# kurtkuehnert/bevy_terrain

Hardware: AMD Instinct MI355X
Metric: terrain tiles/sec preprocessed (16k^2 heightmap) (higher is better)
Workload: dtype f32; 1 GPU; synthetic 16384x16384 fBm R16 heightmap (seed 42), T=512, b=2, lod_count=6: split + pyramid + stitch into 1365 tiles; jobs_in_flight=1, ranks_seen=1, all_gather_bytes_per_rank=0

## Files before the change

bevy_terrain_amd/csrc/bt_fused.hip:

```cpp
#include <cstdio>
#include <cstdlib>
#include <type_traits>

#include "bt_internal.hpp"

namespace bt {

namespace {

constexpr uint32_t kInvalid = 0xFFFFFFFFu;

#include "bt_stitch.hpp"

#ifdef BT_DEBUG_HOOKS
#define BT_ABLATE(A, bits) ((A).ablate & (bits))
#else
#define BT_ABLATE(A, bits) 0u
#endif
constexpr uint32_t kMainRows = 8;
#ifndef BT_DMA_POS
#define BT_DMA_POS 0
#endif

constexpr uint32_t kDmaPos = BT_DMA_POS;
constexpr uint32_t kMaxBorder = 8;

struct MainItem {
    uint32_t side, x, y, atlas_index, raster;
};

struct FusedArgs {
    AttachmentMeta m;
    uint16_t* atlas;
    const RasterDev* rasters;
    const MainItem* items;
    const uint32_t* grids;
    uint32_t grid_lod_lo, grid_lod_hi, grid_sides;
    uint32_t regular, reg_first;
    const TaskDev* seam_tasks;
    uint32_t seam_count, seam_skip;
    uint32_t seam_pull;
    uint32_t tail_extras;
    float tlx, tly, brx, bry;
    uint32_t lod;
    uint32_t levels;
    uint32_t item_count;
    uint32_t groups;
    uint32_t sides;
    uint32_t lds_pitch;
    uint32_t lds_rows;
    uint32_t apron_lods;
    uint32_t rotate_priority;
    uint32_t apron_cols;
    uint32_t prev_zero;
    uint32_t apron_global;
    uint32_t single_buffer;
    uint32_t ablate;
};

__device__ __forceinline__ float unorm16_to_float(uint32_t t) {
    const float x = float(t);
    const float r = 1.0f / 65535.0f;
    const float q0 = x * r;
    const float e = __builtin_fmaf(-q0, 65535.0f, x);
    return __builtin_fmaf(e, r, q0);
}
__device__ __forceinline__ uint32_t float_to_unorm16(float e) {
    const float cl = __builtin_amdgcn_fmed3f(e, 0.0f, 1.0f);
    return uint32_t(0.5f + 65535.0f * cl);
}
__device__ __forceinline__ float mixf(float a, float b, float t) { return a * (1.0f - t) + b * t; }

struct Axis {
    int i0, i1;
    float fr;
};

__host__ __device__ __forceinline__ Axis split_axis(uint32_t r, uint32_t c, uint32_t tile, float scale, float lo, float hi, uint32_t dim) {
    const float tc = float(r) / float(c);
    const float s = (float(tile) + tc) / scale;
    const float u = (s - lo) / (hi - lo);
    const float q = u * float(dim) - 0.5f;
    const float fl = floorf(q);
    Axis a;
    a.fr = q - fl;
    const int i = int(fl);
    const int last = int(dim) - 1;
    const int j = i + 1;
    a.i0 = i < 0 ? 0 : (i > last ? last : i);
    a.i1 = j < 0 ? 0 : (j > last ? last : j);
    return a;
}

__device__ __forceinline__ uint32_t grid_lookup(const FusedArgs& A, uint32_t side, uint32_t lod, int x, int y) {
    const int n = int(1u << lod);
    if (x < 0 || y < 0 || x >= n || y >= n) return kInvalid;
    if (lod < A.grid_lod_lo || lod > A.grid_lod_hi || side >= A.grid_sides) return kInvalid;
    if (A.regular) {
        const uint32_t hi4 = 4u << (2u * A.grid_lod_hi);
        return A.reg_first + side * ((hi4 - (1u << (2u * A.grid_lod_lo))) / 3u) + (hi4 - (4u << (2u * lod))) / 3u + uint32_t(x) * uint32_t(n) + uint32_t(y);
    }
    const uint32_t lo4 = 1u << (2u * A.grid_lod_lo), per_side = ((4u << (2u * A.grid_lod_hi)) - lo4) / 3u;
    const uint32_t off = side * per_side + ((1u << (2u * lod)) - lo4) / 3u;
    return A.grids[off + uint32_t(x) * uint32_t(n) + uint32_t(y)];
}

struct TileNb {
    uint32_t self, n, e, s, w;
};

__device__ __forceinline__ TileNb load_tile_nb(const FusedArgs& A, uint32_t side, uint32_t lod, uint32_t x, uint32_t y) {
    const int ix = int(x), iy = int(y);
    TileNb t;
    t.self = grid_lookup(A, side, lod, ix, iy);
    t.n = grid_lookup(A, side, lod, ix, iy - 1);
    t.e = grid_lookup(A, side, lod, ix + 1, iy);
    t.s = grid_lookup(A, side, lod, ix, iy + 1);
    t.w = grid_lookup(A, side, lod, ix - 1, iy);
    return t;
}

template <bool kCentre = true, typename TT = uint16_t>
__device__ __forceinline__ void push_pixel(const FusedArgs& A, uint32_t side, uint32_t lod, uint32_t tx, uint32_t ty,
                                           uint32_t self_index, uint32_t cx, uint32_t cy, TT v) {
    const uint32_t T = A.m.texture_size, b = A.m.border_size, c = A.m.center_size;
    const uint64_t tile_texels = uint64_t(T) * T;
    TT* atlas = reinterpret_cast<TT*>(A.atlas);
    TT* self = atlas + uint64_t(self_index) * tile_texels;
    if (kCentre) self[uint64_t(b + cy) * T + b + cx] = v;
    const int ex = cx < b ? -1 : (cx >= c - b ? 1 : 0);
    const int ey = cy < b ? -1 : (cy >= c - b ? 1 : 0);
    if (ex == 0 && ey == 0) return;
    const uint32_t o = b + c;
    const int ix = int(tx), iy = int(ty);
    const uint32_t ax = uint32_t(int(b + cx) - ex * int(c)), ay = uint32_t(int(b + cy) - ey * int(c));
    const int nn = int(1u << lod);
    auto cross_face = [&](int x, int y) { return A.seam_pull != 0 && ((x < 0 || x >= nn) != (y < 0 || y >= nn)); };
    if (ex != 0) {
        const uint32_t n = grid_lookup(A, side, lod, ix + ex, iy);
        if (n != kInvalid) {
            atlas[uint64_t(n) * tile_texels + uint64_t(b + cy) * T + ax] = v;
        } else if (cross_face(ix + ex, iy)) {
        } else if (cx == 0 || cx == c - 1) {
            const uint32_t x0 = ex < 0 ? 0u : o;
            for (uint32_t j = 0; j < b; j++) self[uint64_t(b + cy) * T + x0 + j] = v;
        }
    }
    if (ey != 0) {
        const uint32_t n = grid_lookup(A, side, lod, ix, iy + ey);
        if (n != kInvalid) {
            atlas[uint64_t(n) * tile_texels + uint64_t(ay) * T + b + cx] = v;
        } else if (cross_face(ix, iy + ey)) {
        } else if (cy == 0 || cy == c - 1) {
            const uint32_t y0 = ey < 0 ? 0u : o;
            for (uint32_t j = 0; j < b; j++) self[uint64_t(y0 + j) * T + b + cx] = v;
        }
    }
    if (ex != 0 && ey != 0) {
        const uint32_t n = grid_lookup(A, side, lod, ix + ex, iy + ey);
        if (n != kInvalid) {
            atlas[uint64_t(n) * tile_texels + uint64_t(ay) * T + ax] = v;
        } else if (cross_face(ix + ex, iy + ey)) {
        } else if ((cx == 0 || cx == c - 1) && (cy == 0 || cy == c - 1)) {
            const uint32_t x0 = ex < 0 ? 0u : o, y0 = ey < 0 ? 0u : o;
            for (uint32_t j = 0; j < b; j++)
                for (uint32_t i = 0; i < b; i++) self[uint64_t(y0 + j) * T + x0 + i] = v;
        }
    }
}

struct PushNb {
    int ex, ey;
    uint32_t nx, ny, nxy;
    uint32_t skip;
};
__device__ __forceinline__ PushNb push_targets(const FusedArgs& A, uint32_t side, uint32_t lod, uint32_t tx, uint32_t ty, uint32_t cx, uint32_t cy, bool active) {
    const uint32_t b = A.m.border_size, c = A.m.center_size;
    PushNb t{0, 0, kInvalid, kInvalid, kInvalid, 0u};
    if (!active) return t;
    t.ex = cx < b ? -1 : (cx >= c - b ? 1 : 0);
    t.ey = cy < b ? -1 : (cy >= c - b ? 1 : 0);
    if (t.ex != 0) t.nx = grid_lookup(A, side, lod, int(tx) + t.ex, int(ty));
    if (t.ey != 0) t.ny = grid_lookup(A, side, lod, int(tx), int(ty) + t.ey);
    if (t.ex != 0 && t.ey != 0) t.nxy = grid_lookup(A, side, lod, int(tx) + t.ex, int(ty) + t.ey);
    if (A.seam_pull) {
        const int nn = int(1u << lod), x = int(tx) + t.ex, y = int(ty) + t.ey;
        const bool out_x = x < 0 || x >= nn, out_y = y < 0 || y >= nn;
        t.skip = (t.ex != 0 && out_x ? 1u : 0u) | (t.ey != 0 && out_y ? 2u : 0u) | (t.ex != 0 && t.ey != 0 && out_x != out_y ? 4u : 0u);
    }
    return t;
}
template <typename TT = uint16_t>
__device__ __forceinline__ void push_store(const FusedArgs& A, const PushNb& t, uint32_t self_index, uint32_t cx, uint32_t cy, TT v) {
    if (t.ex == 0 && t.ey == 0) return;
    const uint32_t T = A.m.texture_size, b = A.m.border_size, c = A.m.center_size, o = b + c;
    const uint64_t tile_texels = uint64_t(T) * T;
    TT* atlas = reinterpret_cast<TT*>(A.atlas);
    TT* self = atlas + uint64_t(self_index) * tile_texels;
    const uint32_t ax = uint32_t(int(b + cx) - t.ex * int(c)), ay = uint32_t(int(b + cy) - t.ey * int(c));
    if (t.ex != 0) {
        if (t.nx != kInvalid) {
            atlas[uint64_t(t.nx) * tile_texels + uint64_t(b + cy) * T + ax] = v;
        } else if (t.skip & 1u) {
        } else if (cx == 0 || cx == c - 1) {
            const uint32_t x0 = t.ex < 0 ? 0u : o;
            for (uint32_t j = 0; j < b; j++) self[uint64_t(b + cy) * T + x0 + j] = v;
        }
    }
    if (t.ey != 0) {
        if (t.ny != kInvalid) {
            atlas[uint64_t(t.ny) * tile_texels + uint64_t(ay) * T + b + cx] = v;
        } else if (t.skip & 2u) {
        } else if (cy == 0 || cy == c - 1) {
            const uint32_t y0 = t.ey < 0 ? 0u : o;
            for (uint32_t j = 0; j < b; j++) self[uint64_t(y0 + j) * T + b + cx] = v;
        }
    }
    if (t.ex != 0 && t.ey != 0) {
        if (t.nxy != kInvalid) {
            atlas[uint64_t(t.nxy) * tile_texels + uint64_t(ay) * T + ax] = v;
        } else if (t.skip & 4u) {
        } else if ((cx == 0 || cx == c - 1) && (cy == 0 || cy == c - 1)) {
            const uint32_t x0 = t.ex < 0 ? 0u : o, y0 = t.ey < 0 ? 0u : o;
            for (uint32_t j = 0; j < b; j++)
                for (uint32_t i = 0; i < b; i++) self[uint64_t(y0 + j) * T + x0 + i] = v;
        }
    }
}

__device__ __forceinline__ uint32_t downsample4(uint32_t t00, uint32_t t01, uint32_t t10, uint32_t t11) {
    if (t00 != 0 && t01 != 0 && t10 != 0 && t11 != 0) {
        const float value = ((unorm16_to_float(t00) + unorm16_to_float(t01)) + unorm16_to_float(t10)) + unorm16_to_float(t11);
        return float_to_unorm16(value * 0.25f);
    }
    float value = 0.0f, count = 0.0f;
    if (t00 != 0) { value += unorm16_to_float(t00); count += 1.0f; }
    if (t01 != 0) { value += unorm16_to_float(t01); count += 1.0f; }
    if (t10 != 0) { value += unorm16_to_float(t10); count += 1.0f; }
    if (t11 != 0) { value += unorm16_to_float(t11); count += 1.0f; }
    if (count == 0.0f) return 0;
    return float_to_unorm16(value / count);
}

__device__ __forceinline__ float unorm8_to_float(uint32_t t) {
    const float x = float(t), r = 1.0f / 255.0f;
    const float q0 = x * r;
    return __builtin_fmaf(__builtin_fmaf(-q0, 255.0f, x), r, q0);
}
__device__ __forceinline__ uint32_t downsample4_rgba8(uint32_t t00, uint32_t t01, uint32_t t10, uint32_t t11) {
    const uint32_t t[4] = {t00, t01, t10, t11};
    if ((t00 & 0x00FFFFFFu) != 0 && (t01 & 0x00FFFFFFu) != 0 && (t10 & 0x00FFFFFFu) != 0 && (t11 & 0x00FFFFFFu) != 0) {
        uint32_t out = 0;
#pragma unroll
        for (int k = 0; k < 4; k++) {
            const uint32_t sh = 8 * k;
            const float a = float((t00 >> sh) & 0xFFu), bq = float((t01 >> sh) & 0xFFu), cq = float((t10 >> sh) & 0xFFu), d = float((t11 >> sh) & 0xFFu);
            const float r = 1.0f / 255.0f;
            const float sum = ((__builtin_fmaf(a, r, a) + __builtin_fmaf(bq, r, bq)) + __builtin_fmaf(cq, r, cq)) + __builtin_fmaf(d, r, d);
            out |= uint32_t(0.5f + (255.0f / 256.0f) * (sum * 0.25f)) << sh;
        }
        return out;
    }
    float value[4] = {0.0f, 0.0f, 0.0f, 0.0f}, count = 0.0f;
#pragma unroll
    for (int i = 0; i < 4; i++)
        if ((t[i] & 0x00FFFFFFu) != 0) {
#pragma unroll
            for (int k = 0; k < 4; k++) value[k] += unorm8_to_float((t[i] >> (8 * k)) & 0xFFu);
            count += 1.0f;
        }
    if (count == 0.0f) return 0;
    uint32_t out = 0;
#pragma unroll
    for (int k = 0; k < 4; k++) {
        const float e = value[k] / count;
        const float cl = e < 0.0f ? 0.0f : (e > 1.0f ? 1.0f : e);
        out |= uint32_t(floorf(0.5f + 255.0f * cl)) << (8 * k);
    }
    return out;
}

__device__ __forceinline__ uint32_t split_value_slow(const FusedArgs& A, const RasterDev& r, uint32_t tx, uint32_t rx, uint32_t ty,
                                                  uint32_t ry, uint32_t home_index) {
    const float scale = float(1u << A.lod);
    const uint32_t c = A.m.center_size, b = A.m.border_size, T = A.m.texture_size;
    const Axis ax = split_axis(rx, c, tx, scale, A.tlx, A.brx, r.width);
    const Axis ay = split_axis(ry, c, ty, scale, A.tly, A.bry, r.height);
    typedef const uint8_t __attribute__((address_space(1))) * global_bytes;
    typedef const uint16_t __attribute__((address_space(1))) * global_u16;
    const global_u16 row0 = (global_u16)((global_bytes)r.data + uint64_t(ay.i0) * r.pitch);
    const global_u16 row1 = (global_u16)((global_bytes)r.data + uint64_t(ay.i1) * r.pitch);
    const uint32_t t00 = row0[ax.i0], t10 = row0[ax.i1], t01 = row1[ax.i0], t11 = row1[ax.i1];
    if (t00 == 0 || t10 == 0 || t01 == 0 || t11 == 0) {
        if (home_index == kInvalid || A.prev_zero) return 0;
        return A.atlas[uint64_t(home_index) * T * T + uint64_t(b + ry) * T + b + rx];
    }
    const float top = mixf(unorm16_to_float(t00), unorm16_to_float(t10), ax.fr);
    const float bot = mixf(unorm16_to_float(t01), unorm16_to_float(t11), ax.fr);
    return float_to_unorm16(mixf(top, bot, ay.fr));
}

__device__ __forceinline__ uint32_t xcd_remap(uint32_t bid, uint32_t total) {
    const uint32_t q = total / 8u, r = total % 8u, xcd = bid % 8u, i = bid / 8u;
    return (xcd < r ? xcd * (q + 1u) : r * (q + 1u) + (xcd - r) * q) + i;
}

__device__ __forceinline__ int wave_min(int v) {
#pragma unroll
    for (int o = 32; o > 0; o >>= 1) v = min(v, __shfl_xor(v, o));
    return v;
}
__device__ __forceinline__ int wave_max(int v) {
#pragma unroll
    for (int o = 32; o > 0; o >>= 1) v = max(v, __shfl_xor(v, o));
    return v;
}

struct RowParam {
    int y0, y1;
    float fy;
    uint32_t pad;
};

constexpr uint32_t kMaxChunks = 64;
struct MainShared {
    int row_y0[kMaxChunks * kMainRows];
    float2 row_fy[kMaxChunks * kMainRows];
    int win_ymin[kMaxChunks];
    uint32_t win_slots[kMaxChunks];
    RowParam apron[2 * kMaxBorder];
    int xmin, xmax;
    uint32_t pad_[2];
};
static_assert(sizeof(MainShared) % 16 == 0, "LDS carve must stay 16-byte aligned");

struct Texel4 {
    float a0, a1, b0, b1;
    uint32_t za, zb;
};

__device__ __forceinline__ Texel4 convert4(uint32_t ta0, uint32_t ta1, uint32_t tb0, uint32_t tb1) {
    Texel4 r;
    r.a0 = unorm16_to_float(ta0);
    r.a1 = unorm16_to_float(ta1);
    r.b0 = unorm16_to_float(tb0);
    r.b1 = unorm16_to_float(tb1);
    r.za = min(ta0, ta1);
    r.zb = min(tb0, tb1);
    return r;
}

__device__ __forceinline__ void corner_pixels(const FusedArgs& A, uint32_t item_index, uint32_t tid, uint32_t threads) {
    const MainItem it = A.items[item_index];
    const RasterDev raster = A.rasters[it.raster];
    const uint32_t T = A.m.texture_size, b = A.m.border_size, c = A.m.center_size, o = b + c;
    const uint32_t self = grid_lookup(A, it.side, A.lod, int(it.x), int(it.y));
    for (uint32_t t = tid; t < 4 * b * b; t += threads) {
        const uint32_t corner = t / (b * b), i = (t % (b * b)) % b, j = (t % (b * b)) / b;
        const bool left = corner == 0 || corner == 3, top = corner < 2;
        const uint32_t px = left ? i : o + i, py = top ? j : o + j;
        const uint32_t n = grid_lookup(A, it.side, A.lod, int(it.x) + (left ? -1 : 1), int(it.y) + (top ? -1 : 1));
        uint32_t v;
        if (n != kInvalid)
            v = split_value_slow(A, raster, left ? it.x - 1 : it.x + 1, left ? c - b + i : i, top ? it.y - 1 : it.y + 1, top ? c - b + j : j, n);
        else
            v = split_value_slow(A, raster, it.x, left ? 0u : c - 1, it.y, top ? 0u : c - 1, self);
        A.atlas[uint64_t(self) * T * T + py * T + px] = uint16_t(v);
    }
}

template <bool kStaged, bool kGeneric, uint32_t kT, uint32_t kP, bool kDma = false>
__device__ __forceinline__ void fused_main_chunks(const FusedArgs& A, uint32_t item_index, uint32_t k_begin, uint32_t k_end, uint8_t* smem) {
    MainShared& S = *reinterpret_cast<MainShared*>(smem);
    uint16_t* s_buf = reinterpret_cast<uint16_t*>(smem + sizeof(MainShared));
    constexpr bool kFix = kStaged && !kGeneric;
    const bool one_buffer = kDma && kP == 0 && A.single_buffer != 0;
    const uint32_t buf_texels = one_buffer ? 0u : A.lds_rows * (kP ? kP : A.lds_pitch);

    const MainItem it = A.items[item_index];
    const RasterDev raster = A.rasters[it.raster];
    const uint32_t T = kT ? kT : A.m.texture_size, b = A.m.border_size, c = A.m.center_size, o = b + c;
    const uint32_t tid = threadIdx.x;
#ifdef BT_DEBUG_HOOKS
    auto wg_stamp = [&](uint32_t slot) {
        if (BT_ABLATE(A, 134217728u) && tid == 0 && blockIdx.x < 4096u)
            reinterpret_cast<unsigned long long*>(A.atlas + uint64_t(A.m.atlas_size - 1u) * T * T)[16384u + blockIdx.x * 4u + slot] = __builtin_amdgcn_s_memrealtime();
    };
#else
    auto wg_stamp = [&](uint32_t) {};
#endif
    wg_stamp(0);
    const float scale = float(1u << A.lod);
    const uint32_t tile_texels = T * T;
    const uint32_t chunks_per_tile = (c + kMainRows - 1) / kMainRows;

    const TileNb t5 = load_tile_nb(A, it.side, A.lod, it.x, it.y);
    const uint32_t self4 = A.levels >= 2 ? grid_lookup(A, it.side, A.lod - 1, int(it.x >> 1), int(it.y >> 1)) : kInvalid;
    const uint32_t self3 = A.levels >= 3 ? grid_lookup(A, it.side, A.lod - 2, int(it.x >> 2), int(it.y >> 2)) : kInvalid;

    for (uint32_t i = tid; i < (k_end - k_begin) * kMainRows; i += 256u) {
        const uint32_t cr = k_begin * kMainRows + i;
        if (cr < c) {
            const Axis ay = split_axis(cr, c, it.y, scale, A.tly, A.bry, raster.height);
            S.row_y0[i] = ay.i0 | (ay.i1 == ay.i0 ? int(0x80000000u) : 0);
            S.row_fy[i] = float2{ay.fr, 1.0f - ay.fr};
        }
    }
    if (tid >= 32 && tid < 32 + 2 * b) {
        const uint32_t r = tid - 32, k = r % b;
        const bool top = r < b;
        const uint32_t nrow = top ? t5.n : t5.s;
        uint32_t ty, ry;
        if (nrow != kInvalid) { ty = top ? it.y - 1 : it.y + 1; ry = top ? c - b + k : k; } else { ty = it.y; ry = top ? 0u : c - 1; }
        const Axis ay = split_axis(ry, c, ty, scale, A.tly, A.bry, raster.height);
        S.apron[r].y0 = ay.i0;
        S.apron[r].y1 = ay.i1;
        S.apron[r].fy = ay.fr;
        S.apron[r].pad = ry;
    }

    const uint32_t half_c = c / 2, half_b = b / 2;
    const bool is_centre = tid < half_c;
    const bool is_right = !is_centre && tid < half_c + half_b;
    const bool is_left = !is_centre && !is_right && tid < half_c + 2 * half_b;
    const bool is_idle = !is_centre && !is_right && !is_left;
    uint32_t px0 = 0;
    uint32_t txa = it.x, txb = it.x, rxa = 0, rxb = 0;
    if (is_centre) {
        px0 = b + 2 * tid;
        rxa = 2 * tid;
        rxb = 2 * tid + 1;
    } else if (is_right) {
        const uint32_t j = 2 * (tid - half_c);
        px0 = o + j;
        if (t5.e != kInvalid) { txa = txb = it.x + 1; rxa = j; rxb = j + 1; } else { rxa = rxb = c - 1; }
    } else if (is_left) {
        const uint32_t j = 2 * (tid - half_c - half_b);
        px0 = j;
        if (t5.w != kInvalid) { txa = txb = it.x - 1; rxa = c - b + j; rxb = c - b + j + 1; } else { rxa = rxb = 0; }
    }
    const Axis axa = split_axis(rxa, c, txa, scale, A.tlx, A.brx, raster.width);
    const Axis axb = split_axis(rxb, c, txb, scale, A.tlx, A.brx, raster.width);
    const float fxa = axa.fr, fxb = axb.fr, gxa = 1.0f - fxa, gxb = 1.0f - fxb;
    const uint32_t home_col = is_right && t5.e != kInvalid ? t5.e : (is_left && t5.w != kInvalid ? t5.w : t5.self);

    if (tid == half_c + half_b) S.xmin = min(axa.i0, axb.i0);
    if (tid == half_c + half_b - 1) S.xmax = max(axa.i1, axb.i1);
    __syncthreads();
    if (tid < k_end - k_begin) {
        const uint32_t k = k_begin + tid, n = min(kMainRows, c - k * kMainRows);
        const int* y0 = S.row_y0 + tid * kMainRows;
        const int first = y0[0] & 0x7fffffff;
        bool consecutive = n == kMainRows;
        for (uint32_t i = 0; i < n; i++) consecutive = consecutive && y0[i] == first + int(i);
        int lo = first, hi = (y0[n - 1] & 0x7fffffff) + (y0[n - 1] < 0 ? 0 : 1);
        if (!(kDma && kP == 0 && A.apron_global)) {
            if (k == 0) lo = min(lo, S.apron[0].y0);
            if (k == chunks_per_tile - 1) hi = max(hi, S.apron[2 * b - 1].y1);
        }
        S.win_ymin[tid] = lo;
        S.win_slots[tid] = uint32_t(hi - lo + 1) | (consecutive ? 0x80000000u : 0u);
    }
    __syncthreads();

    const int xa = __builtin_amdgcn_readfirstlane(S.xmin) & ~7;
    const uint32_t P = kP ? kP : A.lds_pitch;
    typedef const uint8_t __attribute__((address_space(1))) * global_bytes;
    typedef const uint16_t __attribute__((address_space(1))) * global_u16;
    typedef uint32_t u32x4 __attribute__((ext_vector_type(4)));
    typedef const u32x4 __attribute__((address_space(1))) * global_u4;
    typedef uint16_t u16x2 __attribute__((ext_vector_type(2)));
    const global_bytes data = (global_bytes)raster.data;
    const uint32_t chunks_per_row = P / 8u;
    const uint32_t row_texels = uint32_t(raster.pitch / 2u);
    const bool wide = ((reinterpret_cast<uintptr_t>(raster.data) | raster.pitch) & 15u) == 0;
    constexpr uint32_t kBatch = 4;

    auto chunk_rows = [&](uint32_t k) -> uint32_t { return min(kMainRows, c - k * kMainRows); };
    auto window = [&](uint32_t k, int& ymin, uint32_t& slots) {
        ymin = __builtin_amdgcn_readfirstlane(S.win_ymin[k - k_begin]);
        slots = uint32_t(__builtin_amdgcn_readfirstlane(S.win_slots[k - k_begin])) & 0x7fffffffu;
    };
    uint32_t src_off[kBatch], lds_off[kBatch];
#pragma unroll
    for (uint32_t i = 0; i < kBatch; i++) {
        const uint32_t ch = tid + 256u * i;
        const uint32_t slot = ch / chunks_per_row, kk = ch - slot * chunks_per_row;
        const uint32_t x = min(uint32_t(xa) + 8u * kk, row_texels - 8u);
        src_off[i] = slot * uint32_t(raster.pitch) + x * 2u;
        lds_off[i] = (slot * P + 8u * kk) * 2u;
    }
    const uint32_t safe_off = src_off[0] - (tid / chunks_per_row) * uint32_t(raster.pitch);
    auto stage_issue = [&](int ymin, uint32_t slots, u32x4 (&v)[kBatch]) {
        const global_bytes base = data + uint64_t(uint32_t(ymin)) * raster.pitch;
        const uint32_t bound = slots * P * 2u;
#pragma unroll
        for (uint32_t i = 0; i < kBatch; i++) {
            const global_u4 ptr = (global_u4)(base + (lds_off[i] < bound ? src_off[i] : safe_off));
            v[i] = BT_ABLATE(A, 32768u) ? __builtin_nontemporal_load(ptr) : *ptr;
        }
    };
    auto stage_commit = [&](uint16_t* s_src, uint32_t slots, const u32x4 (&v)[kBatch]) {
        const uint32_t bound = slots * P * 2u;
        uint8_t* s_bytes = reinterpret_cast<uint8_t*>(s_src);
#pragma unroll
        for (uint32_t i = 0; i < kBatch; i++)
            if (lds_off[i] < bound) *reinterpret_cast<u32x4*>(s_bytes + lds_off[i]) = v[i];
    };
    auto stage_narrow = [&](uint16_t* s_src, int ymin, uint32_t slots) {
        for (uint32_t i = tid; i < slots * P; i += 256u) {
            const uint32_t slot = i / P, kk = i - slot * P;
            const uint32_t x = uint32_t(xa) + kk;
            const global_u16 row = (global_u16)(data + uint64_t(ymin + int(slot)) * raster.pitch);
            s_src[i] = x < raster.width ? row[x] : uint16_t(1);
        }
    };

    typedef __attribute__((address_space(3))) uint8_t* lds_bytes;
    const uint32_t dma_lane = tid & 63u;
    const uint32_t dma_off_main = min(uint32_t(xa) * 2u + dma_lane * 16u, uint32_t(raster.pitch) - 16u);
    const uint32_t dma_off_tail = min(uint32_t(xa) * 2u + 1024u + (dma_lane & 1u) * 16u, uint32_t(raster.pitch) - 16u);
    auto dma_issue = [&](uint16_t* s_dst, int ymin, uint32_t slots) {
        static_assert(!kDma || kP == 528 || kP == 0, "the DMA variants: 1056-byte LDS rows, or a run-time pitch");
        const lds_bytes dst = (lds_bytes)reinterpret_cast<uint8_t*>(s_dst);
        for (uint32_t slot = uint32_t(__builtin_amdgcn_readfirstlane(int(tid >> 6))); slot < slots; slot += 4u) {
            const global_bytes row = data + uint64_t(uint32_t(ymin) + slot) * raster.pitch;
            if constexpr (kP == 528) {
                if (BT_ABLATE(A, 32768u))
                    __builtin_amdgcn_global_load_lds((const __attribute__((address_space(1))) void*)(row + dma_off_main),
                                                     (__attribute__((address_space(3))) void*)(dst + slot * (kP * 2u)), 16, 0, 2);
                else
                __builtin_amdgcn_global_load_lds((const __attribute__((address_space(1))) void*)(row + dma_off_main),
                                                 (__attribute__((address_space(3))) void*)(dst + slot * (kP * 2u)), 16, 0, 0);
                if (dma_lane < 2u)
                    __builtin_amdgcn_global_load_lds((const __attribute__((address_space(1))) void*)(row + dma_off_tail),
                                                     (__attribute__((address_space(3))) void*)(dst + slot * (kP * 2u) + 1024u), 16, 0, 0);
            } else {
                const uint32_t row_bytes = P * 2u;
                for (uint32_t piece = 0; piece < row_bytes; piece += 1024u)
                    if (piece + dma_lane * 16u < row_bytes)
                        __builtin_amdgcn_global_load_lds((const __attribute__((address_space(1))) void*)(row + min(uint32_t(xa) * 2u + piece + dma_lane * 16u, uint32_t(raster.pitch) - 16u)),
                                                         (__attribute__((address_space(3))) void*)(dst + slot * row_bytes + piece), 16, 0, 0);
            }
        }
    };

    uint16_t* tile5 = A.atlas + uint64_t(t5.self) * tile_texels;
    uint32_t* tile5_u32 = reinterpret_cast<uint32_t*>(tile5);
    uint16_t* tile4 = A.atlas + uint64_t(self4 == kInvalid ? 0u : self4) * tile_texels;
    uint16_t* tile3 = A.atlas + uint64_t(self3 == kInvalid ? 0u : self3) * tile_texels;
    const uint32_t cx4 = (it.x & 1u) * half_c + tid, cy4_base = (it.y & 1u) * half_c;
    const uint32_t cx3 = (it.x & 3u) * (c / 4) + (tid >> 1), cy3_base = (it.y & 3u) * (c / 4);
    const bool do4 = A.levels >= 2 && !BT_ABLATE(A, 1u), do3 = A.levels >= 3 && !BT_ABLATE(A, 1u);
    auto make_xpush = [&](uint32_t shift, uint32_t self, uint32_t cx, uint32_t& layer, uint32_t& off, uint32_t& count) {
        layer = 0;
        off = 0;
        count = 0;
        if (!is_centre || self == kInvalid) return;
        const bool left = cx < b, right = cx >= c - b;
        if (!left && !right) return;
        const uint32_t n = grid_lookup(A, it.side, A.lod - shift, int(it.x >> shift) + (left ? -1 : 1), int(it.y >> shift));
        const uint32_t j = left ? cx : cx - (c - b);
        if (n != kInvalid) {
            layer = n;
            off = b * T + (left ? o + j : j);
            count = 1;
        } else if (left ? cx == 0 : cx == c - 1) {
            layer = self;
            off = b * T + (left ? 0u : o);
            count = b;
        }
    };
    uint32_t x4_layer, x4_off, x4_count, x3_layer, x3_off, x3_count;
    make_xpush(1, A.levels >= 2 ? self4 : kInvalid, cx4, x4_layer, x4_off, x4_count);
    make_xpush(2, A.levels >= 3 ? self3 : kInvalid, cx3, x3_layer, x3_off, x3_count);
    auto xpush4 = [&](uint32_t cy, uint16_t v) {
        for (uint32_t e = 0; e < x4_count; e++) A.atlas[uint64_t(x4_layer) * tile_texels + x4_off + cy * T + e] = v;
    };
    auto xpush3 = [&](uint32_t cy, uint16_t v) {
        for (uint32_t e = 0; e < x3_count; e++) A.atlas[uint64_t(x3_layer) * tile_texels + x3_off + cy * T + e] = v;
    };
    const uint32_t la0 = uint32_t(axa.i0 - xa), la1 = uint32_t(axa.i1 - xa), lb0 = uint32_t(axb.i0 - xa), lb1 = uint32_t(axb.i1 - xa);

    int ymin = 0;
    uint32_t slots = 0;
    u32x4 pre[kBatch];
    window(k_begin, ymin, slots);
    if constexpr (kDma) {
        dma_issue(s_buf + (k_begin & 1u) * buf_texels, ymin, slots);
    } else if (kStaged && !BT_ABLATE(A, 8u)) {
        if (wide) {
            stage_issue(ymin, slots, pre);
            stage_commit(s_buf + (k_begin & 1u) * buf_texels, slots, pre);
        } else {
            stage_narrow(s_buf + (k_begin & 1u) * buf_texels, ymin, slots);
        }
    }
    if constexpr (kStaged) {
        if (k_begin == 0) corner_pixels(A, item_index, tid, 256u);
    }
    auto chunk_barrier = [&]() {
        if constexpr (kDma) asm volatile("s_waitcnt vmcnt(0)" ::: "memory");
        __syncthreads();
    };
    uint16_t* s_src = s_buf;
    int cur_ymin = 0;
    auto fetch_row = [&](int y) -> Texel4 {
        if constexpr (kStaged) {
            const uint16_t* row = s_src + uint32_t(y - cur_ymin) * P;
            return convert4(row[la0], row[la1], row[lb0], row[lb1]);
        } else {
            const global_u16 row = (global_u16)(data + uint64_t(y) * raster.pitch);
            return convert4(row[axa.i0], row[axa.i1], row[axb.i0], row[axb.i1]);
        }
    };
    auto apron_rows = [&](uint32_t k, auto gtag) {
        constexpr bool kKeep = decltype(gtag)::value;
        if (!((k == 0 || k == chunks_per_tile - 1) && is_centre)) return;
        for (uint32_t r = 0; r < 2 * b; r++) {
            const bool top = r < b;
            if (top ? k != 0 : k != chunks_per_tile - 1) continue;
            const uint32_t kk = r % b, py = top ? kk : o + kk;
            const int y0 = __builtin_amdgcn_readfirstlane(S.apron[r].y0), y1 = __builtin_amdgcn_readfirstlane(S.apron[r].y1);
            const float fy = S.apron[r].fy, gy = 1.0f - fy;
            Texel4 t0, t1;
            if (kDma && kP == 0 && A.apron_global) {
                const global_u16 r0 = (global_u16)(data + uint64_t(y0) * raster.pitch), r1 = (global_u16)(data + uint64_t(y1) * raster.pitch);
                t0 = convert4(r0[axa.i0], r0[axa.i1], r0[axb.i0], r0[axb.i1]);
                t1 = convert4(r1[axa.i0], r1[axa.i1], r1[axb.i0], r1[axb.i1]);
            } else {
                t0 = fetch_row(y0);
                t1 = fetch_row(y1);
            }
            uint32_t va = float_to_unorm16((t0.a0 * gxa + t0.a1 * fxa) * gy + (t1.a0 * gxa + t1.a1 * fxa) * fy);
            uint32_t vb = float_to_unorm16((t0.b0 * gxb + t0.b1 * fxb) * gy + (t1.b0 * gxb + t1.b1 * fxb) * fy);
            if (kKeep && min(min(t0.za, t1.za), min(t0.zb, t1.zb)) == 0) {
                const uint32_t nrow = top ? t5.n : t5.s;
                const uint16_t* h = A.atlas + uint64_t(nrow == kInvalid ? t5.self : nrow) * tile_texels + (b + S.apron[r].pad) * T + b;
                if (A.prev_zero) {
                    if (min(t0.za, t1.za) == 0) va = 0;
                    if (min(t0.zb, t1.zb) == 0) vb = 0;
                } else {
                    if (min(t0.za, t1.za) == 0) va = h[rxa];
                    if (min(t0.zb, t1.zb) == 0) vb = h[rxb];
                }
                asm volatile("" : "+v"(va), "+v"(vb));
            }
            tile5_u32[(py * T + px0) >> 1] = va | (vb << 16);
        }
    };
    auto generic_rows = [&](uint32_t k) {
        const int* row_y0 = S.row_y0 + (k - k_begin) * kMainRows;
        const float2* row_fy = S.row_fy + (k - k_begin) * kMainRows;
        const uint32_t cr0 = k * kMainRows, nrows = chunk_rows(k);
        Texel4 cur{};
        int cur_y = -1;
        for (uint32_t q = 0; q < nrows; q += 4) {
            uint32_t va[4], vb[4];
            uint32_t zany = 1;
#pragma unroll
            for (uint32_t i = 0; i < 4; i++) {
                const int yy = __builtin_amdgcn_readfirstlane(row_y0[q + i]);
                const int y0 = yy & 0x7fffffff, y1 = y0 + (yy < 0 ? 0 : 1);
                const float fy = __builtin_bit_cast(float, __builtin_amdgcn_readfirstlane(__builtin_bit_cast(int, row_fy[q + i].x)));
                const Texel4 top = (y0 == cur_y) ? cur : fetch_row(y0);
                const Texel4 bot = (y1 == y0) ? top : fetch_row(y1);
                cur = bot;
                cur_y = y1;
                const float gy = 1.0f - fy;
                va[i] = float_to_unorm16((top.a0 * gxa + top.a1 * fxa) * gy + (bot.a0 * gxa + bot.a1 * fxa) * fy);
                vb[i] = float_to_unorm16((top.b0 * gxb + top.b1 * fxb) * gy + (bot.b0 * gxb + bot.b1 * fxb) * fy);
                const uint32_t za = min(top.za, bot.za), zb = min(top.zb, bot.zb);
                zany = min(zany, min(za, zb));
                va[i] |= za == 0 ? 0x10000u : 0u;
                vb[i] |= zb == 0 ? 0x10000u : 0u;
            }
            if (zany == 0) {
#pragma unroll
                for (uint32_t i = 0; i < 4; i++) {
                    const uint16_t* h = A.atlas + uint64_t(home_col) * tile_texels + (b + cr0 + q + i) * T + b;
                    if (va[i] & 0x10000u) va[i] = A.prev_zero ? 0u : uint32_t(h[rxa]);
                    if (vb[i] & 0x10000u) vb[i] = A.prev_zero ? 0u : uint32_t(h[rxb]);
                }
            }
            const uint32_t py = b + cr0 + q;
            if (!is_idle) {
#pragma unroll
                for (uint32_t i = 0; i < 4; i++) tile5_u32[((py + i) * T + px0) >> 1] = (va[i] & 0xFFFFu) | (vb[i] << 16);
            }
            if (do4) {
                const uint32_t cy = cr0 + q;
                const uint32_t q0 = downsample4(va[0] & 0xFFFFu, va[1] & 0xFFFFu, vb[0] & 0xFFFFu, vb[1] & 0xFFFFu);
                const uint32_t q1 = downsample4(va[2] & 0xFFFFu, va[3] & 0xFFFFu, vb[2] & 0xFFFFu, vb[3] & 0xFFFFu);
                const uint32_t cy4 = cy4_base + (cy >> 1);
                if (is_centre) {
                    uint16_t* dst = tile4 + (b + cy4) * T + b + cx4;
                    dst[0] = uint16_t(q0);
                    dst[T] = uint16_t(q1);
                }
                if (x4_count) {
                    xpush4(cy4, uint16_t(q0));
                    xpush4(cy4 + 1, uint16_t(q1));
                }
                if (do3) {
                    const uint32_t other0 = __shfl_xor(q0, 1), other1 = __shfl_xor(q1, 1);
                    if (is_centre && (tid & 1u) == 0) {
                        const uint32_t w = downsample4(q0, q1, other0, other1);
                        tile3[(b + cy3_base + (cy >> 2)) * T + b + cx3] = uint16_t(w);
                        if (x3_count) xpush3(cy3_base + (cy >> 2), uint16_t(w));
                    }
                }
            }
        }
    };

    chunk_barrier();
    wg_stamp(1);

    for (uint32_t k = k_begin; k < k_end; k++) {
        const int* row_y0 = S.row_y0 + (k - k_begin) * kMainRows;
        const float2* row_fy = S.row_fy + (k - k_begin) * kMainRows;
        const uint32_t cr0 = k * kMainRows, nrows = chunk_rows(k);
        s_src = s_buf + (k & 1u) * buf_texels;
        cur_ymin = ymin;
        int next_ymin = 0;
        uint32_t next_slots = 0;
        const bool more = k + 1 < k_end;
        if (more) {
            window(k + 1, next_ymin, next_slots);
            if constexpr (kDma) {
                if (BT_ABLATE(A, 2048u)) __builtin_amdgcn_s_setprio(3);
                if (kDmaPos == 0 && !one_buffer) dma_issue(s_buf + ((k + 1) & 1u) * buf_texels, next_ymin, next_slots);
            }
            else if (kStaged && wide && !BT_ABLATE(A, 8u)) stage_issue(next_ymin, next_slots, pre);
        }

        if (A.rotate_priority) {
            switch (((blockIdx.x / 8u) / 32u + k) & 3u) {
                case 0: __builtin_amdgcn_s_setprio(0); break;
                case 1: __builtin_amdgcn_s_setprio(1); break;
                case 2: __builtin_amdgcn_s_setprio(2); break;
                default: __builtin_amdgcn_s_setprio(3); break;
            }
        }
#ifdef BT_DEBUG_HOOKS
#define BT_FUSED_DEBUG_CHUNK_PROBES
#include "bt_fused_debug.inc"
#undef BT_FUSED_DEBUG_CHUNK_PROBES
#endif
        apron_rows(k, std::integral_constant<bool, true>{});

#ifdef BT_DEBUG_HOOKS
#define BT_FUSED_DEBUG_SKELETON_STORES
#include "bt_fused_debug.inc"
#undef BT_FUSED_DEBUG_SKELETON_STORES
#endif
        if (!BT_ABLATE(A, 16u)) {
            if constexpr (kStaged && !kGeneric) {
                typedef float f2 __attribute__((ext_vector_type(2)));
                const f2 gx = {gxa, gxb}, fx = {fxa, fxb};
                const f2 kr = {1.0f / 65535.0f, 1.0f / 65535.0f}, kn = {65535.0f / 65536.0f, 65535.0f / 65536.0f}, khalf = {0.5f, 0.5f};
                const f2 kzero = {0.0f, 0.0f}, knq = {0.25f * (65535.0f / 65536.0f), 0.25f * (65535.0f / 65536.0f)};
                auto conv2 = [&](uint32_t ta, uint32_t tb) -> f2 {
                    const f2 x = {float(ta), float(tb)};
                    return __builtin_elementwise_fma(x, kr, x);
                };
                auto quantise = [&](f2 v) -> f2 { return khalf + kn * v; };
                auto quantise_quarter = [&](f2 s) -> f2 { return khalf + knq * s; };
                const uint32_t cy4_first = cy4_base + (cr0 >> 1), cy3_first = cy3_base + (cr0 >> 2);
                if (kMainRows == 8 && __builtin_amdgcn_readfirstlane(int(S.win_slots[k - k_begin])) < 0) {
                    const uint16_t* base = s_src + uint32_t(__builtin_amdgcn_readfirstlane(row_y0[0]) - cur_ymin) * P;
                    const uint16_t *pa0 = base + la0, *pa1 = base + la1, *pb0 = base + lb0, *pb1 = base + lb1;
                    const float2* fyt = row_fy;
                    u16x2 ta = {pa0[0], pb0[0]}, tb = {pa1[0], pb1[0]};
                    u16x2 na = {pa0[P], pb0[P]}, nb = {pa1[P], pb1[P]};
                    auto conv2p = [&](u16x2 t) -> f2 { return conv2(t.x, t.y); };
                    f2 hprev = conv2p(ta) * gx + conv2p(tb) * fx;
                    uint32_t q[4];
                    u16x2 zmin[2] = {__builtin_elementwise_min(ta, tb), u16x2{0xFFFFu, 0xFFFFu}};
                    u16x2 z[5] = {zmin[0], zmin[0], zmin[0], zmin[0], zmin[0]};
                    uint32_t zq[2] = {1u, 1u};
                    uint32_t sink[8] = {0u, 0u, 0u, 0u, 0u, 0u, 0u, 0u};
                    uint32_t* dst5 = tile5_u32 + (((b + cr0) * T + px0) >> 1);
#pragma unroll
                    for (uint32_t quad = 0; quad < 2; quad++) {
                        uint32_t ua[4], ub[4];
#pragma unroll
                        for (uint32_t i = 0; i < 4; i++) {
                            const uint32_t r = 4 * quad + i;
                            ta = na;
                            tb = nb;
                            if (r + 2 <= kMainRows) {
                                na = u16x2{pa0[(r + 2) * P], pb0[(r + 2) * P]};
                                nb = u16x2{pa1[(r + 2) * P], pb1[(r + 2) * P]};
                            }
                            if (kDma && kDmaPos == 10 + r && more) dma_issue(s_buf + ((k + 1) & 1u) * buf_texels, next_ymin, next_slots);
                            if constexpr (kFix) {
                                const u16x2 zrow = __builtin_elementwise_min(ta, tb);
                                zmin[quad] = __builtin_elementwise_min(zmin[quad], zrow);
                                if (quad == 0 && i == 3) zmin[1] = zrow;
                                if (quad == 1 && i == 0) z[0] = z[4];
                                z[i + 1] = zrow;
                            }
                            const f2 hnew = conv2p(ta) * gx + conv2p(tb) * fx;
                            const float2 wy = fyt[r];
                            const f2 fy2 = {wy.x, wy.x}, gy2 = {wy.y, wy.y};
                            const f2 w = quantise(hprev * gy2 + hnew * fy2);
                            hprev = hnew;
                            ua[i] = uint32_t(w.x);
                            ub[i] = uint32_t(w.y);
                        }
                        if constexpr (kFix) {
                            zq[quad] = min(uint32_t(zmin[quad].x), uint32_t(zmin[quad].y));
                            if (__builtin_expect(zq[quad] == 0, 0)) {
                                const uint16_t* h = A.atlas + uint64_t(home_col) * tile_texels + (b + cr0 + 4 * quad) * T + b;
                                if (A.prev_zero) {
#pragma unroll
                                    for (uint32_t i = 0; i < 4; i++) {
                                        if (min(z[i].x, z[i + 1].x) == 0) ua[i] = 0;
                                        if (min(z[i].y, z[i + 1].y) == 0) ub[i] = 0;
                                    }
                                } else if (BT_ABLATE(A, 1073741824u)) {
#pragma unroll
                                    for (uint32_t i = 0; i < 4; i++) {
                                        if (min(z[i].x, z[i + 1].x) == 0) ua[i] = 0;
                                        if (min(z[i].y, z[i + 1].y) == 0) ub[i] = 0;
                                        asm volatile("global_load_ushort %0, %1, off" : "=v"(sink[2 * i]) : "v"(h + i * T + rxa) : "memory");
                                        asm volatile("global_load_ushort %0, %1, off" : "=v"(sink[2 * i + 1]) : "v"(h + i * T + rxb) : "memory");
                                    }
                                } else {
#pragma unroll
                                    for (uint32_t i = 0; i < 4; i++) {
                                        if (min(z[i].x, z[i + 1].x) == 0) ua[i] = h[i * T + rxa];
                                        if (min(z[i].y, z[i + 1].y) == 0) ub[i] = h[i * T + rxb];
                                    }
                                }
#pragma unroll
                                for (uint32_t i = 0; i < 4; i++) asm volatile("" : "+v"(ua[i]), "+v"(ub[i]));
                            }
                        }
                        if (!is_idle && !BT_ABLATE(A, 2u)) {
#pragma unroll
                            for (uint32_t i = 0; i < 4; i++) {
                                if (BT_ABLATE(A, 8192u)) __builtin_nontemporal_store(ua[i] | (ub[i] << 16), &dst5[(4 * quad + i) * (T / 2)]);
                                else dst5[(4 * quad + i) * (T / 2)] = ua[i] | (ub[i] << 16);
                            }
                        }
                        if (kDma && kDmaPos == quad + 1 && more) dma_issue(s_buf + ((k + 1) & 1u) * buf_texels, next_ymin, next_slots);
                        if (do4) {
                            const f2 sum = ((conv2(ua[0], ua[2]) + conv2(ua[1], ua[3])) + conv2(ub[0], ub[2])) + conv2(ub[1], ub[3]);
                            const f2 wq = quantise_quarter(sum);
                            q[2 * quad] = uint32_t(wq.x);
                            q[2 * quad + 1] = uint32_t(wq.y);
                            if (kFix && __builtin_expect(zq[quad] == 0, 0)) {
                                const uint32_t ca = min(ua[0], 1u) + min(ua[1], 1u) + min(ub[0], 1u) + min(ub[1], 1u), cb = min(ua[2], 1u) + min(ua[3], 1u) + min(ub[2], 1u) + min(ub[3], 1u);
                                const f2 d = {sum.x / float(max(ca, 1u)), sum.y / float(max(cb, 1u))};
                                const f2 wv = khalf + kn * d;
                                q[2 * quad] = uint32_t(wv.x);
                                q[2 * quad + 1] = uint32_t(wv.y);
                            }
                        }
                    }
                    if (do4) {
                        uint32_t both[4];
#pragma unroll
                        for (uint32_t j = 0; j < 4; j++)
                            both[j] = q[j] | (uint32_t(__builtin_amdgcn_update_dpp(0, int(q[j]), 0xB1, 0xf, 0xf, true)) << 16);
                        if (is_centre && (tid & 1u) == 0 && !BT_ABLATE(A, 4u)) {
                            uint32_t* dst = reinterpret_cast<uint32_t*>(tile4 + (b + cy4_first) * T + b + cx4);
#pragma unroll
                            for (uint32_t j = 0; j < 4; j++) {
                                if (BT_ABLATE(A, 16384u)) __builtin_nontemporal_store(both[j], &dst[j * (T / 2)]);
                                else dst[j * (T / 2)] = both[j];
                            }
                        }
                        if (x4_count && !BT_ABLATE(A, 4u)) {
                            uint16_t* t = A.atlas + uint64_t(x4_layer) * tile_texels + x4_off + cy4_first * T;
#pragma unroll
                            for (uint32_t j = 0; j < 4; j++) t[j * T] = uint16_t(q[j]);
                            if (x4_count > 1)
                                for (uint32_t e = 1; e < x4_count; e++)
#pragma unroll
                                    for (uint32_t j = 0; j < 4; j++) t[j * T + e] = uint16_t(q[j]);
                        }
                        if (do3) {
                            const bool even = (tid & 1u) == 0;
                            const f2 c02 = conv2(q[0], q[2]), c13 = conv2(q[1], q[3]);
                            const f2 colsum = c02 + c13;
                            auto swap_pair = [](float v) -> float {
                                return __builtin_bit_cast(float, __builtin_amdgcn_update_dpp(0, __builtin_bit_cast(int, v), 0xB1, 0xf, 0xf, true));
                            };
                            const float recv1 = swap_pair(even ? colsum.y : c02.x), recv2 = swap_pair(c13.x);
                            const float sa = even ? colsum.x : recv1, sb = even ? recv1 : c02.y, sc = even ? recv2 : c13.y;
                            const float s3 = (sa + sb) + sc;
                            uint32_t w3 = uint32_t(0.5f + (0.25f * (65535.0f / 65536.0f)) * s3);
                            if constexpr (kFix) {
                                const uint32_t m0 = even ? q[0] : q[2], m1 = even ? q[1] : q[3];
                                const uint32_t p0 = (even ? both[0] : both[2]) >> 16, p1 = (even ? both[1] : both[3]) >> 16;
                                if (__builtin_expect(min(min(m0, m1), min(p0, p1)) == 0, 0)) w3 = even ? downsample4(m0, m1, p0, p1) : downsample4(p0, p1, m0, m1);
                            }
                            const uint32_t row3 = (b + cy3_first + (even ? 0u : 1u)) * T;
                            if (is_centre && !BT_ABLATE(A, 64u)) tile3[row3 + b + cx3] = uint16_t(w3);
                            if (x3_count && !BT_ABLATE(A, 64u)) {
                                uint16_t* t = A.atlas + uint64_t(x3_layer) * tile_texels + x3_off + (cy3_first + (even ? 0u : 1u)) * T;
                                t[0] = uint16_t(w3);
                                if (x3_count > 1)
                                    for (uint32_t e = 1; e < x3_count; e++) t[e] = uint16_t(w3);
                            }
                        }
                    }
                    if (BT_ABLATE(A, 1073741824u)) {
                        asm volatile("s_waitcnt vmcnt(0)" ::: "memory");
#pragma unroll
                        for (uint32_t i = 0; i < 8; i++) asm volatile("" ::"v"(sink[i]));
                    }
                } else {
                uint32_t zrow = 1;
                auto hblend = [&](int y) -> f2 {
                    const uint16_t* row = s_src + uint32_t(y - cur_ymin) * P;
                    const uint32_t r0 = row[la0], r1 = row[lb0], r2 = row[la1], r3 = row[lb1];
                    if constexpr (kFix) zrow = min(min(r0, r1), min(r2, r3));
                    const f2 left = conv2(r0, r1), right = conv2(r2, r3);
                    return left * gx + right * fx;
                };
                f2 hcur = kzero;
                int hy = -1;
                uint32_t zcur = 1;
                for (uint32_t q = 0; q < nrows; q += 4) {
                    uint32_t ua[4], ub[4];
                    uint32_t zq = 1;
#pragma unroll
                    for (uint32_t i = 0; i < 4; i++) {
                        const int yy = __builtin_amdgcn_readfirstlane(row_y0[q + i]);
                        const int y0 = yy & 0x7fffffff, y1 = y0 + (yy < 0 ? 0 : 1);
                        const float fy = __builtin_bit_cast(float, __builtin_amdgcn_readfirstlane(__builtin_bit_cast(int, row_fy[q + i].x)));
                        f2 top = hcur;
                        uint32_t ztop = zcur;
                        if (y0 != hy) {
                            top = hblend(y0);
                            ztop = zrow;
                        }
                        f2 bot = top;
                        uint32_t zbot = ztop;
                        if (y1 != y0) {
                            bot = hblend(y1);
                            zbot = zrow;
                        }
                        hcur = bot;
                        zcur = zbot;
                        hy = y1;
                        zq = min(zq, min(ztop, zbot));
                        const f2 fy2 = {fy, fy}, gy2 = {1.0f - fy, 1.0f - fy};
                        const f2 w = quantise(top * gy2 + bot * fy2);
                        ua[i] = uint32_t(w.x);
                        ub[i] = uint32_t(w.y);
                    }
                    const bool fix = kFix && zq == 0;
                    if (fix) {
                        const uint16_t* h = A.atlas + uint64_t(home_col) * tile_texels + (b + cr0 + q) * T + b;
#pragma unroll
                        for (uint32_t i = 0; i < 4; i++) {
                            const int yy = row_y0[q + i];
                            const uint16_t* r0 = s_src + uint32_t((yy & 0x7fffffff) - cur_ymin) * P;
                            const uint16_t* r1 = r0 + (yy < 0 ? 0u : P);
                            if (min(min(r0[la0], r0[la1]), min(r1[la0], r1[la1])) == 0) ua[i] = A.prev_zero ? 0u : uint32_t(h[i * T + rxa]);
                            if (min(min(r0[lb0], r0[lb1]), min(r1[lb0], r1[lb1])) == 0) ub[i] = A.prev_zero ? 0u : uint32_t(h[i * T + rxb]);
                        }
#pragma unroll
                        for (uint32_t i = 0; i < 4; i++) asm volatile("" : "+v"(ua[i]), "+v"(ub[i]));
                    }
                    const uint32_t py = b + cr0 + q;
                    if (!is_idle && !BT_ABLATE(A, 2u)) {
#pragma unroll
                        for (uint32_t i = 0; i < 4; i++) tile5_u32[((py + i) * T + px0) >> 1] = ua[i] | (ub[i] << 16);
                    }
                    if (kDma && kDmaPos != 0 && q == ((kDmaPos == 1 || kDmaPos >= 10) ? 0u : (nrows > 4 ? 4u : 0u)) && more) dma_issue(s_buf + ((k + 1) & 1u) * buf_texels, next_ymin, next_slots);
                    if (do4) {
                        const f2 s = ((conv2(ua[0], ua[2]) + conv2(ua[1], ua[3])) + conv2(ub[0], ub[2])) + conv2(ub[1], ub[3]);
                        const f2 wq = quantise_quarter(s);
                        uint32_t q0 = uint32_t(wq.x), q1 = uint32_t(wq.y);
                        if (fix) {
                            const uint32_t ca = min(ua[0], 1u) + min(ua[1], 1u) + min(ub[0], 1u) + min(ub[1], 1u), cb = min(ua[2], 1u) + min(ua[3], 1u) + min(ub[2], 1u) + min(ub[3], 1u);
                            const f2 d = {s.x / float(max(ca, 1u)), s.y / float(max(cb, 1u))};
                            const f2 wv = khalf + kn * d;
                            q0 = uint32_t(wv.x);
                            q1 = uint32_t(wv.y);
                        }
                        const uint32_t cy = cr0 + q, cy4 = cy4_base + (cy >> 1);
                        if (is_centre) {
                            uint16_t* dst = tile4 + (b + cy4) * T + b + cx4;
                            dst[0] = uint16_t(q0);
                            dst[T] = uint16_t(q1);
                        }
                        if (x4_count) {
                            xpush4(cy4, uint16_t(q0));
                            xpush4(cy4 + 1, uint16_t(q1));
                        }
                        if (do3) {
                            const uint32_t other0 = __shfl_xor(q0, 1), other1 = __shfl_xor(q1, 1);
                            if (is_centre && (tid & 1u) == 0) {
                                const f2 mine = conv2(q0, q1), theirs = conv2(other0, other1);
                                const float s3 = ((mine.x + mine.y) + theirs.x) + theirs.y;
                                uint32_t w3 = uint32_t(0.5f + (0.25f * (65535.0f / 65536.0f)) * s3);
                                if (kFix && min(min(q0, q1), min(other0, other1)) == 0) w3 = downsample4(q0, q1, other0, other1);
                                const uint32_t cy3 = cy3_base + (cy >> 2);
                                tile3[(b + cy3) * T + b + cx3] = uint16_t(w3);
                                if (x3_count) xpush3(cy3, uint16_t(w3));
                            }
                        }
                    }
                }
                }
            } else {
                generic_rows(k);
            }
        }

        if (!more) break;
        if (kStaged && !kDma && !BT_ABLATE(A, 8u)) {
            uint16_t* s_next = s_buf + ((k + 1) & 1u) * buf_texels;
            if (wide) stage_commit(s_next, next_slots, pre);
            else stage_narrow(s_next, next_ymin, next_slots);
        }
        ymin = next_ymin;
        slots = next_slots;
        if constexpr (kDma && kP == 0) {
            if (one_buffer) {
                __syncthreads();
                dma_issue(s_buf, next_ymin, next_slots);
            }
        }
        chunk_barrier();
    }
    wg_stamp(2);
#ifdef BT_DEBUG_HOOKS
    if (BT_ABLATE(A, 134217728u) && tid == 0)
        reinterpret_cast<unsigned long long*>(A.atlas + uint64_t(A.m.atlas_size - 1u) * tile_texels)[item_index * 8u + 4u] = __builtin_amdgcn_s_memrealtime();
#endif
    wg_stamp(3);
}

template <bool kStaged, bool kGeneric, uint32_t kT, uint32_t kP, bool kDma = false>
__global__ __launch_bounds__(256) __attribute__((amdgpu_waves_per_eu(4, 4))) void fused_main_kernel(FusedArgs A) {
    extern __shared__ __attribute__((aligned(16))) uint8_t smem[];
    const uint32_t work = BT_ABLATE(A, 1024u) ? blockIdx.x : xcd_remap(blockIdx.x, gridDim.x);
    const uint32_t chunks_per_tile = (A.m.center_size + kMainRows - 1) / kMainRows;
    const uint32_t part = work % A.groups;
    const uint32_t k_begin = part * chunks_per_tile / A.groups, k_end = (part + 1) * chunks_per_tile / A.groups;
    if (k_begin >= k_end) return;
#ifdef BT_DEBUG_HOOKS
#define BT_FUSED_DEBUG_ENTRY_PRIORITY
#include "bt_fused_debug.inc"
#undef BT_FUSED_DEBUG_ENTRY_PRIORITY
#endif
    fused_main_chunks<kStaged, kGeneric, kT, kP, kDma>(A, work / A.groups, k_begin, k_end, smem);
}

__global__ __launch_bounds__(64) void fused_corner_kernel(FusedArgs A) { corner_pixels(A, blockIdx.x, threadIdx.x, blockDim.x); }

constexpr uint32_t kApronPairsPerThread = 4;
__device__ __forceinline__ void tail_apron_rows(const FusedArgs& A, uint32_t side, uint32_t e) {
    const uint32_t T = A.m.texture_size, b = A.m.border_size, c = A.m.center_size, o = b + c;
    const uint32_t pairs = b * T, per_block = 256u * kApronPairsPerThread, blocks_per_tile = (pairs + per_block - 1u) / per_block;
    for (uint32_t k = 0; k < A.apron_lods; k++) {
        const uint32_t lod = A.lod + k, n = 1u << lod, blocks = n * n * blocks_per_tile;
        if (e >= blocks) {
            e -= blocks;
            continue;
        }
        const uint32_t tile = e / blocks_per_tile, i0 = (e % blocks_per_tile) * per_block + threadIdx.x;
        const uint32_t tx = tile / n, ty = tile % n;
        const uint32_t self = grid_lookup(A, side, lod, int(tx), int(ty));
        if (self == kInvalid) return;
        uint32_t v[kApronPairsPerThread][2], dst[kApronPairsPerThread];
        bool live[kApronPairsPerThread];
#pragma unroll
        for (uint32_t q = 0; q < kApronPairsPerThread; q++) {
            const uint32_t i = i0 + 256u * q;
            live[q] = i < pairs;
            const uint32_t ii = live[q] ? i : 0u;
            const uint32_t r = ii / (T / 2u), px = 2u * (ii % (T / 2u)), py = r < b ? r : c + r;
            const int rx = px < b ? -1 : (px >= o ? 1 : 0), ry = r < b ? -1 : 1;
            if (A.seam_skip) {
                const bool out_x = int(tx) + rx < 0 || int(tx) + rx >= int(n), out_y = int(ty) + ry < 0 || int(ty) + ry >= int(n);
                if (out_x != out_y) live[q] = false;
            }
            const uint32_t nb = grid_lookup(A, side, lod, int(tx) + rx, int(ty) + ry);
#pragma unroll
            for (uint32_t h = 0; h < 2; h++) {
                const uint32_t x = px + h;
                const uint32_t sx = nb != kInvalid ? uint32_t(int(x) - rx * int(c)) : min(max(x, b), o - 1u);
                const uint32_t sy = nb != kInvalid ? uint32_t(int(py) - ry * int(c)) : min(max(py, b), o - 1u);
                v[q][h] = A.atlas[uint64_t(nb != kInvalid ? nb : self) * T * T + sy * T + sx];
            }
            dst[q] = py * T + px;
        }
#pragma unroll
        for (uint32_t q = 0; q < kApronPairsPerThread; q++)
            if (live[q]) *reinterpret_cast<uint32_t*>(A.atlas + uint64_t(self) * T * T + dst[q]) = v[q][0] | (v[q][1] << 16);
        return;
    }
}

__device__ __forceinline__ uint32_t tail_apron_texels_per_tile(const FusedArgs& A) {
    return 2u * A.m.border_size * A.m.texture_size + (A.apron_cols ? 2u * A.m.border_size * A.m.center_size : 0u);
}
__device__ __forceinline__ void tail_aprons_rgba8(const FusedArgs& A, uint32_t side, uint32_t e) {
    const uint32_t T = A.m.texture_size, b = A.m.border_size, c = A.m.center_size, o = b + c;
    const uint32_t per_tile = tail_apron_texels_per_tile(A), blocks_per_tile = (per_tile + 255u) / 256u;
    uint32_t* atlas = reinterpret_cast<uint32_t*>(A.atlas);
    for (uint32_t k = 0; k < A.apron_lods; k++) {
        const uint32_t lod = A.lod + k, n = 1u << lod, blocks = n * n * blocks_per_tile;
        if (e >= blocks) {
            e -= blocks;
            continue;
        }
        const uint32_t tile = e / blocks_per_tile, i = (e % blocks_per_tile) * 256u + threadIdx.x;
        if (i >= per_tile) return;
        const uint32_t tx = tile / n, ty = tile % n;
        const uint32_t self = grid_lookup(A, side, lod, int(tx), int(ty));
        if (self == kInvalid) return;
        uint32_t px, py;
        if (i < 2u * b * T) {
            const uint32_t r = i / T;
            px = i % T;
            py = r < b ? r : c + r;
        } else {
            const uint32_t j = i - 2u * b * T, kk = j % (2u * b);
            px = kk < b ? kk : c + kk;
            py = b + j / (2u * b);
        }
        const int rx = px < b ? -1 : (px >= o ? 1 : 0), ry = py < b ? -1 : (py >= o ? 1 : 0);
        if (A.seam_skip) {
            const bool out_x = int(tx) + rx < 0 || int(tx) + rx >= int(n), out_y = int(ty) + ry < 0 || int(ty) + ry >= int(n);
            if (out_x != out_y) return;
        }
        const uint32_t nb = grid_lookup(A, side, lod, int(tx) + rx, int(ty) + ry);
        const uint32_t sx = nb != kInvalid ? uint32_t(int(px) - rx * int(c)) : min(max(px, b), o - 1u);
        const uint32_t sy = nb != kInvalid ? uint32_t(int(py) - ry * int(c)) : min(max(py, b), o - 1u);
        atlas[uint64_t(self) * T * T + py * T + px] = atlas[uint64_t(nb != kInvalid ? nb : self) * T * T + sy * T + sx];
        return;
    }
}

typedef float tail_f2 __attribute__((ext_vector_type(2)));
typedef uint16_t tail_u16x2 __attribute__((ext_vector_type(2)));
__device__ __forceinline__ tail_f2 tail_conv2(uint32_t a, uint32_t bq) {
    const tail_f2 x = {float(a), float(bq)}, kr = {1.0f / 65535.0f, 1.0f / 65535.0f};
    return __builtin_elementwise_fma(x, kr, x);
}
__device__ __forceinline__ void down_pair_r16(uint32_t a_top, uint32_t a_bot, uint32_t b_top, uint32_t b_bot, uint32_t& qa, uint32_t& qb) {
    const tail_f2 khalf = {0.5f, 0.5f}, kn = {65535.0f / 65536.0f, 65535.0f / 65536.0f}, knq = {0.25f * (65535.0f / 65536.0f), 0.25f * (65535.0f / 65536.0f)};
    const tail_u16x2 one = {1, 1};
    const tail_u16x2 at = __builtin_bit_cast(tail_u16x2, a_top), ab = __builtin_bit_cast(tail_u16x2, a_bot), bt2 = __builtin_bit_cast(tail_u16x2, b_top), bb = __builtin_bit_cast(tail_u16x2, b_bot);
    const tail_u16x2 m = __builtin_elementwise_min(__builtin_elementwise_min(at, ab), __builtin_elementwise_min(bt2, bb));
    const tail_f2 sum = ((tail_conv2(a_top & 0xFFFFu, b_top & 0xFFFFu) + tail_conv2(a_bot & 0xFFFFu, b_bot & 0xFFFFu)) + tail_conv2(a_top >> 16, b_top >> 16)) + tail_conv2(a_bot >> 16, b_bot >> 16);
    tail_f2 w = khalf + knq * sum;
    if (__builtin_expect(m.x == 0 || m.y == 0, 0)) {
        const tail_u16x2 ca = __builtin_elementwise_min(at, one) + __builtin_elementwise_min(ab, one), cb = __builtin_elementwise_min(bt2, one) + __builtin_elementwise_min(bb, one);
        const tail_f2 d = {sum.x / float(max(uint32_t(ca.x) + uint32_t(ca.y), 1u)), sum.y / float(max(uint32_t(cb.x) + uint32_t(cb.y), 1u))};
        w = khalf + kn * d;
    }
    qa = uint32_t(w.x);
    qb = uint32_t(w.y);
}
__device__ __forceinline__ uint32_t down_one_r16(uint32_t t00, uint32_t t01, uint32_t t10, uint32_t t11) {
    const float r = 1.0f / 65535.0f;
    const float x00 = float(t00), x01 = float(t01), x10 = float(t10), x11 = float(t11);
    const float sum = ((__builtin_fmaf(x00, r, x00) + __builtin_fmaf(x01, r, x01)) + __builtin_fmaf(x10, r, x10)) + __builtin_fmaf(x11, r, x11);
    float w = 0.5f + (0.25f * (65535.0f / 65536.0f)) * sum;
    if (__builtin_expect(min(min(t00, t01), min(t10, t11)) == 0, 0)) {
        const uint32_t count = min(t00, 1u) + min(t01, 1u) + min(t10, 1u) + min(t11, 1u);
        w = 0.5f + (65535.0f / 65536.0f) * (sum / float(max(count, 1u)));
    }
    return uint32_t(w);
}

template <typename TT>
__device__ __forceinline__ uint32_t tail_down(uint32_t t00, uint32_t t01, uint32_t t10, uint32_t t11) {
    if constexpr (std::is_same<TT, uint16_t>::value) return down_one_r16(t00, t01, t10, t11);
    else return downsample4_rgba8(t00, t01, t10, t11);
}
template <int K, typename TT>
__device__ __forceinline__ uint32_t pull_value(const FusedArgs& A, uint32_t side, uint32_t lod, uint32_t mx, uint32_t my) {
    if constexpr (K == 0) {
        const uint32_t T = A.m.texture_size, b = A.m.border_size, c = A.m.center_size;
        const uint32_t tx = mx / c, ty = my / c;
        const uint32_t idx = grid_lookup(A, side, lod, int(tx), int(ty));
        if (idx == kInvalid) return 0u;
        return reinterpret_cast<const TT*>(A.atlas)[uint64_t(idx) * T * T + uint64_t(b + my - ty * c) * T + b + mx - tx * c];
    } else {
        const uint32_t t00 = pull_value<K - 1, TT>(A, side, lod + 1u, 2u * mx, 2u * my), t01 = pull_value<K - 1, TT>(A, side, lod + 1u, 2u * mx, 2u * my + 1u);
        const uint32_t t10 = pull_value<K - 1, TT>(A, side, lod + 1u, 2u * mx + 1u, 2u * my), t11 = pull_value<K - 1, TT>(A, side, lod + 1u, 2u * mx + 1u, 2u * my + 1u);
        return tail_down<TT>(t00, t01, t10, t11);
    }
}

template <typename TT, uint32_t kPack>
__device__ __forceinline__ void stitch_region_pull(const FusedArgs& A, const TaskDev& task) {
    const uint32_t Tsz = A.m.texture_size, b = A.m.border_size, c = A.m.center_size, o = b + c;
    const uint32_t region = uint32_t(__ffs(int(task.regions))) - 1u;
    const uint32_t x0 = (region == 0u || region == 2u) ? b : ((region == 1u || region == 5u || region == 6u) ? o : 0u);
    const uint32_t y0 = (region == 1u || region == 3u) ? b : ((region == 2u || region == 6u || region == 7u) ? o : 0u);
    const uint32_t w = (region == 0u || region == 2u) ? c : b, h = (region == 1u || region == 3u) ? c : b;
    const int rx = (region == 1u || region == 5u || region == 6u) ? 1 : ((region == 3u || region == 4u || region == 7u) ? -1 : 0);
    const int ry = (region == 2u || region == 6u || region == 7u) ? 1 : ((region == 0u || region == 4u || region == 5u) ? -1 : 0);
    const uint32_t other = task.rel_side[region], nx = task.rel_index[region] >> 16, ny = task.rel_index[region] & 0xFFFFu;
    const uint32_t levels = task.raster & 0xFFu, part = (task.raster >> 8) & 0xFFu, parts = max(1u, task.raster >> 16);
    const uint32_t count = (w / kPack) * h, share = (count + parts - 1u) / parts, i_end = min(count, (part + 1u) * share);
    const uint32_t in_lod = task.lod + levels, cn = c >> levels;
    for (uint32_t i = part * share + threadIdx.x; i < i_end; i += 256u) {
        const uint32_t px = x0 + kPack * (i % (w / kPack)), py = y0 + i / (w / kPack);
        if (py >= A.m.row_limit) continue;
        uint32_t v[kPack];
#pragma unroll
        for (uint32_t e = 0; e < kPack; e++) {
            const uint2 q = project_to_side(uint32_t(int(px + e) - rx * int(c)), uint32_t(int(py) - ry * int(c)), Tsz, task.side, other);
            const uint32_t mx = nx * c + (q.x - b), my = ny * c + (q.y - b);
            if (BT_ABLATE(A, 2147483648u)) {
                v[e] = 0;
            } else if (levels <= 2u && (c & 3u) == 0) {
                const uint32_t tx = mx / cn, ty = my / cn;
                const uint32_t idx = grid_lookup(A, other, in_lod, int(tx), int(ty));
                const TT* src = reinterpret_cast<const TT*>(A.atlas) + uint64_t(idx == kInvalid ? 0u : idx) * Tsz * Tsz + uint64_t(b + ((my - ty * cn) << levels)) * Tsz + b + ((mx - tx * cn) << levels);
                const uint32_t keep = idx == kInvalid ? 0u : 0xFFFFFFFFu;
                if (levels == 1u) {
                    const uint32_t t00 = src[0], t01 = src[Tsz], t10 = src[1], t11 = src[Tsz + 1u];
                    v[e] = tail_down<TT>(t00 & keep, t01 & keep, t10 & keep, t11 & keep);
                } else {
                    uint32_t t[4][4];
#pragma unroll
                    for (uint32_t dy = 0; dy < 4; dy++)
#pragma unroll
                        for (uint32_t dx = 0; dx < 4; dx++) t[dy][dx] = uint32_t(src[dy * Tsz + dx]) & keep;
                    auto two = [&](uint32_t dx, uint32_t dy) -> uint32_t { return tail_down<TT>(t[dy][dx], t[dy + 1][dx], t[dy][dx + 1], t[dy + 1][dx + 1]); };
                    v[e] = tail_down<TT>(two(0u, 0u), two(0u, 2u), two(2u, 0u), two(2u, 2u));
                }
            } else {
                v[e] = levels == 1u ? pull_value<1, TT>(A, other, task.lod, mx, my) : levels == 2u ? pull_value<2, TT>(A, other, task.lod, mx, my) : pull_value<3, TT>(A, other, task.lod, mx, my);
            }
        }
        TT* dst = reinterpret_cast<TT*>(A.atlas) + uint64_t(task.atlas_index) * Tsz * Tsz + uint64_t(py) * Tsz + px;
        if (BT_ABLATE(A, 4194304u) && (v[0] | v[kPack - 1]) != 0x12345u) continue;
        if constexpr (kPack == 2) *reinterpret_cast<uint32_t*>(dst) = v[0] | (v[1] << 16);
        else *dst = TT(v[0]);
    }
}

template <uint32_t kFormat, bool kRegular>
__global__ __launch_bounds__(256) void fused_tail_kernel(FusedArgs A_in) {
    FusedArgs A = A_in;
    A.regular = kRegular ? 1u : 0u;
    constexpr bool kR16 = kFormat == BT_FORMAT_R16;
    using TT = typename std::conditional<kR16, uint16_t, uint32_t>::type;
    const uint32_t nx = ((1u << A.lod) * A.m.center_size + 63u) / 64u, per_side_m = nx * nx, per_side_a = A.tail_extras;
    const uint32_t total_m = A.sides * per_side_m, total_a = A.sides * per_side_a, chunk_m = (total_m + 7u) / 8u, chunk_a = (total_a + 7u) / 8u;
    const uint32_t chunk_s = (A.seam_count + 7u) / 8u, chunk_e = chunk_s + chunk_a;
    uint32_t side, block_x, block_y;
    {
        const uint32_t xcd = blockIdx.x % 8u, j = blockIdx.x / 8u;
        if (j < chunk_e) {
            if (BT_ABLATE(A, 268435456u)) return;
            if (j < chunk_s) {
                const uint32_t f = j * 8u + xcd;
                if (f < A.seam_count) {
                    const bool pulled = A.seam_tasks[f].raster != 0u;
                    if constexpr (kR16) {
                        const bool pairs = (A.m.border_size & 1u) == 0 && (A.m.texture_size & 1u) == 0;
                        if (pulled) {
                            if (pairs) stitch_region_pull<uint16_t, 2>(A, A.seam_tasks[f]);
                            else stitch_region_pull<uint16_t, 1>(A, A.seam_tasks[f]);
                        } else if (pairs) stitch_region_body<uint16_t, 2>(A.m, A.atlas, A.seam_tasks[f]);
                        else stitch_region_body<uint16_t, 1>(A.m, A.atlas, A.seam_tasks[f]);
                    } else {
                        if (pulled) stitch_region_pull<uint32_t, 1>(A, A.seam_tasks[f]);
                        else stitch_region_body<uint32_t, 1>(A.m, A.atlas, A.seam_tasks[f]);
                    }
                }
                return;
            }
            const uint32_t id = xcd * chunk_a + (j - chunk_s);
            if (id >= total_a) return;
            side = id / per_side_a;
            const uint32_t e = id - side * per_side_a;
            if constexpr (kR16) tail_apron_rows(A, side, e);
            else tail_aprons_rgba8(A, side, e);
            return;
        }
        const uint32_t id = xcd * chunk_m + (j - chunk_e);
        if (id >= total_m) return;
        side = id / per_side_m;
        const uint32_t r = id - side * per_side_m;
        block_y = r / nx;
        block_x = r - block_y * nx;
    }
    const uint32_t T = A.m.texture_size, b = A.m.border_size, c = A.m.center_size;
    const uint32_t tile_texels = T * T;
    const uint32_t size = (1u << A.lod) * c;
    const uint32_t tx = threadIdx.x & 15u, ty = threadIdx.x >> 4;
    const uint32_t gx = block_x * 64u + 4u * tx, gy = block_y * 64u + 4u * ty;
    const bool active = gx < size && gy < size;
    const uint32_t tile_x = gx / c, tile_y = gy / c, rem_x = gx - tile_x * c, rem_y = gy - tile_y * c;
    const uint32_t rx1 = ((tile_x & 1u) * c + rem_x) >> 1, ry1 = ((tile_y & 1u) * c + rem_y) >> 1;
    TT* atlas = reinterpret_cast<TT*>(A.atlas);
    auto down = [](uint32_t t00, uint32_t t01, uint32_t t10, uint32_t t11) -> uint32_t {
        if constexpr (kR16) return down_one_r16(t00, t01, t10, t11);
        else return downsample4_rgba8(t00, t01, t10, t11);
    };

    uint32_t t[4][4];
#pragma unroll
    for (int r = 0; r < 4; r++)
#pragma unroll
        for (int k = 0; k < 4; k++) t[r][k] = 0;
    uint32_t idx = kInvalid, self1 = kInvalid, self2 = kInvalid, self3 = kInvalid;
    if (active) {
        idx = grid_lookup(A, side, A.lod, int(tile_x), int(tile_y));
        self1 = grid_lookup(A, side, A.lod - 1, int(tile_x >> 1), int(tile_y >> 1));
        if (A.levels >= 2) self2 = grid_lookup(A, side, A.lod - 2, int(tile_x >> 2), int(tile_y >> 2));
        if (A.levels >= 3) self3 = grid_lookup(A, side, A.lod - 3, int(tile_x >> 3), int(tile_y >> 3));
    }
    const bool pre = (b & 1u) == 0;
    const PushNb nb1 = push_targets(A, side, A.lod - 1, tile_x >> 1, tile_y >> 1, rx1, ry1, active && pre);
    if (active) {
        if (idx != kInvalid && !BT_ABLATE(A, 33554432u)) {
            const TT* p = atlas + uint64_t(idx) * tile_texels + (b + rem_y) * T + b + rem_x;
#pragma unroll
            for (int r = 0; r < 4; r++) {
                if constexpr (kR16) {
                    const uint2 w = *reinterpret_cast<const uint2 __attribute__((aligned(4)))*>(p + r * T);
                    t[r][0] = w.x;
                    t[r][1] = w.y;
                } else {
                    if ((b & 1u) == 0) {
                        const uint2 lo = *reinterpret_cast<const uint2*>(p + r * T), hi = *reinterpret_cast<const uint2*>(p + r * T + 2);
                        t[r][0] = lo.x;
                        t[r][1] = lo.y;
                        t[r][2] = hi.x;
                        t[r][3] = hi.y;
                    } else {
#pragma unroll
                        for (int k = 0; k < 4; k++) t[r][k] = p[r * T + k];
                    }
                }
            }
        }
    }
    uint32_t q[2][2];
#pragma unroll
    for (int r = 0; r < 2; r++) {
        if constexpr (kR16) {
            down_pair_r16(t[2 * r][0], t[2 * r + 1][0], t[2 * r][1], t[2 * r + 1][1], q[r][0], q[r][1]);
        } else {
#pragma unroll
            for (int k = 0; k < 2; k++) q[r][k] = down(t[2 * r][2 * k], t[2 * r + 1][2 * k], t[2 * r][2 * k + 1], t[2 * r + 1][2 * k + 1]);
        }
    }
    if (active) {
        const uint32_t self = self1;
        if (self != kInvalid && !BT_ABLATE(A, 1073741824u)) {
            TT* centre = atlas + uint64_t(self) * tile_texels + (b + ry1) * T + b + rx1;
#pragma unroll
            for (int r = 0; r < 2; r++) {
                if constexpr (kR16) {
                    *reinterpret_cast<uint32_t*>(centre + r * T) = q[r][0] | (q[r][1] << 16);
                } else {
                    centre[r * T] = q[r][0];
                    centre[r * T + 1] = q[r][1];
                }
#pragma unroll
                for (int k = 0; k < 2; k++) {
                    if (BT_ABLATE(A, 536870912u)) continue;
                    if (pre) push_store<TT>(A, nb1, self, rx1 + k, ry1 + r, TT(q[r][k]));
                    else push_pixel<false, TT>(A, side, A.lod - 1, tile_x >> 1, tile_y >> 1, self, rx1 + k, ry1 + r, TT(q[r][k]));
                }
            }
        }
    }
    if (A.levels < 2 || BT_ABLATE(A, 67108864u)) return;
    const uint32_t v2 = down(q[0][0], q[1][0], q[0][1], q[1][1]);
    if (active) {
        const uint32_t self = self2;
        if (self != kInvalid)
            push_pixel<true, TT>(A, side, A.lod - 2, tile_x >> 2, tile_y >> 2, self, ((tile_x & 3u) * c + rem_x) >> 2, ((tile_y & 3u) * c + rem_y) >> 2, TT(v2));
    }
    if (A.levels < 3) return;
    const uint32_t right = __shfl_down(v2, 1), below = __shfl_down(v2, 16), diag = __shfl_down(v2, 17);
    if (active && ((tx | ty) & 1u) == 0) {
        const uint32_t v3 = down(v2, below, right, diag);
        const uint32_t self = self3;
        if (self != kInvalid)
            push_pixel<true, TT>(A, side, A.lod - 3, tile_x >> 3, tile_y >> 3, self, ((tile_x & 7u) * c + rem_x) >> 3, ((tile_y & 7u) * c + rem_y) >> 3, TT(v3));
    }
}



__device__ __forceinline__ uint32_t float_to_unorm8(float e) {
    const float cl = e < 0.0f ? 0.0f : (e > 1.0f ? 1.0f : e);
    return uint32_t(floorf(0.5f + 255.0f * cl));
}
struct H4 {
    float h[4];
    bool valid;
};
__device__ __forceinline__ H4 hrow_rgba8(uint32_t t0, uint32_t t1, float fx) {
    H4 o;
    o.valid = (t0 & 0xFFu) != 0 && (t1 & 0xFFu) != 0;
#pragma unroll
    for (uint32_t k = 0; k < 4; k++) o.h[k] = mixf(unorm8_to_float((t0 >> (8 * k)) & 0xFFu), unorm8_to_float((t1 >> (8 * k)) & 0xFFu), fx);
    return o;
}
__device__ __forceinline__ uint32_t vmix_rgba8(const H4& top, const H4& bot, float fy) {
    uint32_t out = 0;
#pragma unroll
    for (uint32_t k = 0; k < 4; k++) out |= float_to_unorm8(mixf(top.h[k], bot.h[k], fy)) << (8 * k);
    return out;
}
__device__ __forceinline__ H4 hrow_rgba8_scaled(uint32_t t0, uint32_t t1, float fx) {
    H4 o;
    o.valid = (t0 & 0xFFu) != 0 && (t1 & 0xFFu) != 0;
    const float gx = 1.0f - fx;
#pragma unroll
    for (uint32_t k = 0; k < 4; k++) {
        const float a = float((t0 >> (8 * k)) & 0xFFu), bb = float((t1 >> (8 * k)) & 0xFFu);
        o.h[k] = __builtin_fmaf(a, 1.0f / 255.0f, a) * gx + __builtin_fmaf(bb, 1.0f / 255.0f, bb) * fx;
    }
    return o;
}
__device__ __forceinline__ uint32_t vmix_rgba8_scaled(const H4& top, const H4& bot, float fy) {
    const float gy = 1.0f - fy;
    uint32_t out = 0;
#pragma unroll
    for (uint32_t k = 0; k < 4; k++) out |= uint32_t(0.5f + (255.0f / 256.0f) * (top.h[k] * gy + bot.h[k] * fy)) << (8 * k);
    return out;
}
typedef const uint8_t __attribute__((address_space(1))) * global_bytes_t;
typedef const uint32_t __attribute__((address_space(1))) * global_u32_t;

__device__ __forceinline__ uint32_t rgba8_value_slow(const FusedArgs& A, const RasterDev& r, uint32_t tx, uint32_t rx, uint32_t ty, uint32_t ry,
                                                     uint32_t home_index) {
    const float scale = float(1u << A.lod);
    const uint32_t c = A.m.center_size, b = A.m.border_size, T = A.m.texture_size;
    const Axis ax = split_axis(rx, c, tx, scale, A.tlx, A.brx, r.width);
    const Axis ay = split_axis(ry, c, ty, scale, A.tly, A.bry, r.height);
    const global_u32_t row0 = (global_u32_t)((global_bytes_t)r.data + uint64_t(ay.i0) * r.pitch);
    const global_u32_t row1 = (global_u32_t)((global_bytes_t)r.data + uint64_t(ay.i1) * r.pitch);
    const H4 top = hrow_rgba8(row0[ax.i0], row0[ax.i1], ax.fr), bot = hrow_rgba8(row1[ax.i0], row1[ax.i1], ax.fr);
    if (!(top.valid && bot.valid)) {
        if (home_index == kInvalid || A.prev_zero) return 0;
        return reinterpret_cast<const uint32_t*>(A.atlas)[uint64_t(home_index) * T * T + uint64_t(b + ry) * T + b + rx];
    }
    return vmix_rgba8(top, bot, ay.fr);
}

__device__ __forceinline__ Axis split_axis_pow2(uint32_t r, uint32_t c, uint32_t tile, float inv_scale, float lo, float hi, uint32_t dim) {
    const float tc = float(r) / float(c);
    const float s = (float(tile) + tc) * inv_scale;
    const float w = hi - lo;
    const float u = w == 1.0f ? s - lo : (s - lo) / w;
    const float q = u * float(dim) - 0.5f;
    const float fl = floorf(q);
    Axis a;
    a.fr = q - fl;
    const int i = int(fl);
    const int last = int(dim) - 1;
    const int j = i + 1;
    a.i0 = i < 0 ? 0 : (i > last ? last : i);
    a.i1 = j < 0 ? 0 : (j > last ? last : j);
    return a;
}

typedef float direct_f2 __attribute__((ext_vector_type(2)));
struct H4p {
    direct_f2 lo, hi;
};
__device__ __forceinline__ H4p conv_rgba8_scaled(uint32_t t) {
    const direct_f2 kr = {1.0f / 255.0f, 1.0f / 255.0f};
    const direct_f2 x01 = {float(t & 0xFFu), float((t >> 8) & 0xFFu)}, x23 = {float((t >> 16) & 0xFFu), float(t >> 24)};
    return H4p{__builtin_elementwise_fma(x01, kr, x01), __builtin_elementwise_fma(x23, kr, x23)};
}
__device__ __forceinline__ H4p hrow_rgba8_packed(uint32_t t0, uint32_t t1, float fx) {
    const direct_f2 f2x = {fx, fx}, g2x = {1.0f - fx, 1.0f - fx};
    const H4p a = conv_rgba8_scaled(t0), bq = conv_rgba8_scaled(t1);
    return H4p{a.lo * g2x + bq.lo * f2x, a.hi * g2x + bq.hi * f2x};
}
__device__ __forceinline__ uint32_t vmix_rgba8_packed(const H4p& top, const H4p& bot, float fy) {
    const direct_f2 f2y = {fy, fy}, g2y = {1.0f - fy, 1.0f - fy}, kn = {255.0f / 256.0f, 255.0f / 256.0f}, khalf = {0.5f, 0.5f};
    const direct_f2 lo = khalf + kn * (top.lo * g2y + bot.lo * f2y), hi = khalf + kn * (top.hi * g2y + bot.hi * f2y);
    return uint32_t(lo.x) | (uint32_t(lo.y) << 8) | (uint32_t(hi.x) << 16) | (uint32_t(hi.y) << 24);
}
__device__ __forceinline__ uint32_t vmix_rgba8_weights(const H4p& top, const H4p& bot, float fy, float gy) {
    const direct_f2 f2y = {fy, fy}, g2y = {gy, gy}, kn = {255.0f / 256.0f, 255.0f / 256.0f}, khalf = {0.5f, 0.5f};
    const direct_f2 lo = khalf + kn * (top.lo * g2y + bot.lo * f2y), hi = khalf + kn * (top.hi * g2y + bot.hi * f2y);
    return uint32_t(lo.x) | (uint32_t(lo.y) << 8) | (uint32_t(hi.x) << 16) | (uint32_t(hi.y) << 24);
}
__device__ __forceinline__ uint32_t downsample4_rgba8_half(uint32_t t00, uint32_t t01, uint32_t t10, uint32_t t11, uint32_t sh) {
    const direct_f2 kr = {1.0f / 255.0f, 1.0f / 255.0f}, knq = {0.25f * (255.0f / 256.0f), 0.25f * (255.0f / 256.0f)}, khalf = {0.5f, 0.5f};
    auto conv = [&](uint32_t t) -> direct_f2 {
        const uint32_t u = t >> sh;
        const direct_f2 x = {float(u & 0xFFu), float((u >> 8) & 0xFFu)};
        return __builtin_elementwise_fma(x, kr, x);
    };
    const direct_f2 sum = ((conv(t00) + conv(t01)) + conv(t10)) + conv(t11);
    const direct_f2 w = khalf + knq * sum;
    return uint32_t(w.x) | (uint32_t(w.y) << 8);
}
template <int kCtrl>
__device__ __forceinline__ uint32_t quad_dpp(uint32_t v) {
    return uint32_t(__builtin_amdgcn_update_dpp(0, int(v), kCtrl, 0xf, 0xf, true));
}

constexpr uint32_t kDirectRows = 4, kDirectMaxBlocks = 16;

template <bool kRep, bool kSkips = false>
__global__ __launch_bounds__(256) __attribute__((amdgpu_waves_per_eu(4, 4))) void fused_direct_rgba8_kernel(FusedArgs A) {
    static_assert(!(kRep && kSkips), "a job's source is coarser or finer than its tile grid, not both");
    constexpr uint32_t kRows = kDirectRows;
    const uint32_t T = A.m.texture_size, b = A.m.border_size, c = A.m.center_size;
    const uint32_t blocks_per_tile = (c + kRows - 1) / kRows;
    const uint32_t nb = A.groups, wgs_per_tile = (blocks_per_tile + nb - 1) / nb;
    const uint32_t work = xcd_remap(blockIdx.x, gridDim.x);
    const MainItem it = A.items[work / wgs_per_tile];
    const uint32_t blk_begin = (work % wgs_per_tile) * nb, blk_end = min(blk_begin + nb, blocks_per_tile);
    const uint32_t row_begin = blk_begin * kRows, row_end = min(blk_end * kRows, c);
    const RasterDev raster = A.rasters[it.raster];
    const float scale = float(1u << A.lod), inv_scale = 1.0f / scale;
    const uint32_t tid = threadIdx.x;
    uint32_t* atlas = reinterpret_cast<uint32_t*>(A.atlas);
    const uint32_t tile_texels = T * T;
    uint32_t* tile = atlas + uint64_t(it.atlas_index) * tile_texels;
#ifdef BT_DEBUG_HOOKS
    auto stamp = [&](uint32_t slot) {
        if (BT_ABLATE(A, 134217728u) && tid == 0)
            reinterpret_cast<unsigned long long*>(atlas + uint64_t(A.m.atlas_size - 1u) * tile_texels)[work * 8u + slot] = __builtin_amdgcn_s_memrealtime();
    };
#else
    auto stamp = [&](uint32_t) {};
#endif
    stamp(0);
    const uint32_t self4 = A.levels >= 2 ? grid_lookup(A, it.side, A.lod - 1, int(it.x >> 1), int(it.y >> 1)) : kInvalid;
    const uint32_t self3 = A.levels >= 3 ? grid_lookup(A, it.side, A.lod - 2, int(it.x >> 2), int(it.y >> 2)) : kInvalid;

    struct BlockInfo {
        int chain, y_first, y_last;
        uint32_t byte_lo, byte_hi;
        int rep;
        int skip;
        int pad[1];
    };
    __shared__ Axis s_ay[kDirectMaxBlocks * kRows];
    __shared__ float2 s_wy[kDirectMaxBlocks * kRows];
    __shared__ BlockInfo s_blk[kDirectMaxBlocks + 2];
    for (uint32_t i = tid; i < row_end - row_begin; i += 256u) {
        const Axis a = split_axis_pow2(row_begin + i, c, it.y, inv_scale, A.tly, A.bry, raster.height);
        s_ay[i] = a;
        s_wy[i] = float2{a.fr, 1.0f - a.fr};
    }
    __syncthreads();
    if (tid < kDirectMaxBlocks + 2) {
        BlockInfo bi = BlockInfo{0, 0, -1, 0u, 0u, 0, 0, {0}};
        if (blk_begin + tid < blk_end && (blk_begin + tid) * kRows + kRows <= c) {
            const Axis* ay = s_ay + tid * kRows;
            bool ok = true;
            int chain = 0x100, rep = 0, skip = 0, skips = 0;
            for (uint32_t r = 0; ok && r < kRows; r++) {
                const int d = ay[r].i1 - ay[r].i0;
                ok = d == 0 || d == 1;
                if (r == 0 || ay[r].i0 == ay[r - 1].i1) chain |= d << r;
                else if (kRep && ay[r].i0 == ay[r - 1].i0 && ay[r].i1 == ay[r - 1].i1) rep |= 1 << r;
                else if (kSkips && ay[r].i0 == ay[r - 1].i1 + 1 && skips < 2) {
                    chain |= d << r;
                    skip |= 1 << r;
                    skips++;
                } else ok = false;
            }
            const uint64_t bytes = uint64_t(uint32_t(ay[0].i0)) * raster.pitch;
            if (ok) bi = BlockInfo{chain, ay[0].i0, ay[kRows - 1].i1, uint32_t(bytes), uint32_t(bytes >> 32), rep, skip, {0}};
        }
        s_blk[tid] = bi;
    }
    __syncthreads();
    const global_bytes_t data = (global_bytes_t)raster.data;
    typedef uint8_t __attribute__((address_space(1))) * global_wbytes_t;
    typedef uint32_t __attribute__((address_space(1))) * global_wu32_t;
    const global_wbytes_t tile_bytes = (global_wbytes_t)tile;
    const global_wbytes_t base4 = (global_wbytes_t)(atlas + uint64_t(self4 == kInvalid ? 0u : self4) * tile_texels + (b + (it.y & 1u) * (c / 2u)) * T + b + (it.x & 1u) * (c / 2u));
    const global_wbytes_t base3 = (global_wbytes_t)(atlas + uint64_t(self3 == kInvalid ? 0u : self3) * tile_texels + (b + (it.y & 3u) * (c / 4u)) * T + b + (it.x & 3u) * (c / 4u));
    const bool narrow = raster.pitch <= (1ull << 28);

    stamp(1);
    const uint32_t c_lanes = (c + 3u) & ~3u;
    const uint32_t last_cx0 = (c_lanes - 1u) / 256u * 256u;
    const bool aprons_in_sweep = last_cx0 + 256u >= c + 2u * b;
    const uint32_t prio_step = max(1u, (last_cx0 / 256u + 1u) * (blk_end - blk_begin) / 4u);
    uint32_t prio_left = prio_step, prio_level = 0;
    __builtin_amdgcn_s_setprio(3);
    for (uint32_t cx0 = 0; cx0 < c_lanes || (aprons_in_sweep && cx0 <= last_cx0); cx0 += 256u) {
        const uint32_t cx = cx0 + tid;
        const bool active = cx < c;
        const bool apron_lane = aprons_in_sweep && cx0 == last_cx0 && !active && cx - c < 2u * b;
        const bool used = active || apron_lane;
        uint32_t home = it.atlas_index, home_col = cx, store_px = b + cx;
        Axis ax = Axis{0, 0, 0.0f};
        if (active) {
            ax = split_axis_pow2(cx, c, it.x, inv_scale, A.tlx, A.brx, raster.width);
        } else if (apron_lane) {
            const uint32_t k = cx - c;
            const int rx = k < b ? -1 : 1;
            store_px = k < b ? k : c + k;
            const uint32_t n = grid_lookup(A, it.side, A.lod, int(it.x) + rx, int(it.y));
            if (n != kInvalid) {
                home = n;
                home_col = uint32_t(int(store_px) - int(b) - rx * int(c));
                ax = split_axis_pow2(home_col, c, uint32_t(int(it.x) + rx), inv_scale, A.tlx, A.brx, raster.width);
            } else {
                home_col = k < b ? 0u : c - 1u;
                ax = split_axis_pow2(home_col, c, it.x, inv_scale, A.tlx, A.brx, raster.width);
            }
        }
        const uint32_t half_sh = (tid & 1u) * 16u;
        const uint32_t off0 = uint32_t(ax.i0) * 4u, off1 = uint32_t(ax.i1) * 4u;
        uint32_t lo0[kRows + 1], lo1[kRows + 1], so[kRows];
#pragma unroll
        for (uint32_t j = 0; j <= kRows; j++) {
            lo0[j] = off0 + j * uint32_t(raster.pitch);
            lo1[j] = off1 + j * uint32_t(raster.pitch);
            asm volatile("" : "+v"(lo0[j]), "+v"(lo1[j]));
        }
#pragma unroll
        for (uint32_t r = 0; r < kRows; r++) {
            so[r] = (store_px + r * T) * 4u;
            asm volatile("" : "+v"(so[r]));
        }
        uint32_t l4 = (cx >> 1) * 4u, l3 = (cx >> 2) * 4u;
        asm volatile("" : "+v"(l4), "+v"(l3));

        uint32_t set_a0[kRows + 1], set_a1[kRows + 1], set_b0[kRows + 1], set_b1[kRows + 1];
        uint32_t extra_a[4] = {0u, 0u, 0u, 0u}, extra_b[4] = {0u, 0u, 0u, 0u};
        BlockInfo info_a, info_b;
        H4p carry_top = H4p{{0.0f, 0.0f}, {0.0f, 0.0f}};
        uint32_t carry_z = 0;
        int carry_row = -1;
        auto block_info = [&](uint32_t blk) -> BlockInfo {
            const BlockInfo* v = s_blk + (blk - blk_begin);
            return BlockInfo{__builtin_amdgcn_readfirstlane(v->chain), __builtin_amdgcn_readfirstlane(v->y_first), __builtin_amdgcn_readfirstlane(v->y_last),
                             uint32_t(__builtin_amdgcn_readfirstlane(int(v->byte_lo))), uint32_t(__builtin_amdgcn_readfirstlane(int(v->byte_hi))),
                             kRep ? __builtin_amdgcn_readfirstlane(v->rep) : 0, kSkips ? __builtin_amdgcn_readfirstlane(v->skip) : 0, {0}};
        };
        auto request = [&](const BlockInfo& bi, uint32_t (&d0)[kRows + 1], uint32_t (&d1)[kRows + 1], uint32_t (&extra)[4]) {
            global_bytes_t rowp = data + (uint64_t(bi.byte_lo) | uint64_t(bi.byte_hi) << 32);
            global_bytes_t xrow0 = rowp, xrow1 = rowp;
            if (BT_ABLATE(A, 8u)) {
#pragma unroll
                for (uint32_t j = 0; j <= kRows; j++) {
                    d0[j] = 0x01010101u * (tid + j + 1u) | 1u;
                    d1[j] = 0x01010101u * (tid + j + 2u) | 1u;
                }
            } else if (__builtin_expect(bi.chain == 0x10F && bi.skip == 0 && narrow, 1)) {
#pragma unroll
                for (uint32_t j = 0; j <= kRows; j++)
                    asm volatile("global_load_dword %0, %2, %4\n\tglobal_load_dword %1, %3, %4" : "=&v"(d0[j]), "=&v"(d1[j]) : "v"(lo0[j]), "v"(lo1[j]), "s"(rowp));
            } else {
#pragma unroll
                for (uint32_t j = 0; j <= kRows; j++) {
                    asm volatile("global_load_dword %0, %2, %4\n\tglobal_load_dword %1, %3, %4" : "=&v"(d0[j]), "=&v"(d1[j]) : "v"(off0), "v"(off1), "s"(rowp));
                    if (kSkips && j >= 1 && j < kRows && ((uint32_t(bi.skip) >> j) & 1u)) {
                        rowp += raster.pitch;
                        if ((uint32_t(bi.skip) & ((1u << j) - 1u)) == 0) xrow0 = rowp; else xrow1 = rowp;
                    }
                    rowp += (uint32_t(bi.chain) >> j) & 1u ? raster.pitch : 0u;
                }
            }
            if constexpr (kSkips) {
                if (bi.skip != 0) {
                    extra[0] = *(global_u32_t)(xrow0 + off0);
                    extra[1] = *(global_u32_t)(xrow0 + off1);
                    extra[2] = *(global_u32_t)(xrow1 + off0);
                    extra[3] = *(global_u32_t)(xrow1 + off1);
                }
            }
        };
        auto arrived = [&](uint32_t j, uint32_t& t0, uint32_t& t1) {
            switch (j) {
                case 0: asm volatile("s_waitcnt vmcnt(18)" : "+v"(t0), "+v"(t1)); break;
                case 1: asm volatile("s_waitcnt vmcnt(16)" : "+v"(t0), "+v"(t1)); break;
                case 2: asm volatile("s_waitcnt vmcnt(14)" : "+v"(t0), "+v"(t1)); break;
                case 3: asm volatile("s_waitcnt vmcnt(12)" : "+v"(t0), "+v"(t1)); break;
                default: asm volatile("s_waitcnt vmcnt(10)" : "+v"(t0), "+v"(t1)); break;
            }
        };
        static_assert(kRows == 4, "arrived() counts 2 x (kRows + 1) loads per request");
        auto block = [&](uint32_t blk, BlockInfo& bi, uint32_t (&raw0)[kRows + 1], uint32_t (&raw1)[kRows + 1], uint32_t (&extra)[4]) {
            if (--prio_left == 0) {
                prio_left = prio_step;
                prio_level++;
                if (prio_level == 1u) __builtin_amdgcn_s_setprio(2);
                else if (prio_level == 2u) __builtin_amdgcn_s_setprio(1);
                else __builtin_amdgcn_s_setprio(0);
            }
            const uint32_t cr0 = blk * kRows, nrows = min(kRows, c - cr0);
            const Axis* ay_blk = s_ay + (blk - blk_begin) * kRows;
            uint32_t out[kRows];
#pragma unroll
            for (uint32_t r = 0; r < kRows; r++) out[r] = 0;
            const bool chained = bi.chain != 0;
            bool fast = chained;
            uint32_t z = 1;
            if (__builtin_expect(chained, 1)) {
                const float2* wy = s_wy + (blk - blk_begin) * kRows;
                H4p top;
                if (__builtin_expect(carry_row == bi.y_first, 1)) {
                    z = carry_z;
                    top = carry_top;
                } else {
                    arrived(0, raw0[0], raw1[0]);
                    z = min(raw0[0] & 0xFFu, raw1[0] & 0xFFu);
                    top = hrow_rgba8_packed(raw0[0], raw1[0], ax.fr);
                }
                if constexpr (!kRep) {
                    const uint32_t x_first0 = extra[0], x_first1 = extra[1], x_second0 = extra[2], x_second1 = extra[3];
#pragma unroll
                    for (uint32_t r = 0; r < kRows; r++) {
                        arrived(r + 1, raw0[r + 1], raw1[r + 1]);
                        const uint32_t z_row = min(raw0[r + 1] & 0xFFu, raw1[r + 1] & 0xFFu);
                        z = min(z, z_row);
                        const H4p bot = hrow_rgba8_packed(raw0[r + 1], raw1[r + 1], ax.fr);
                        if constexpr (kSkips) {
                            if (r > 0 && ((uint32_t(bi.skip) >> r) & 1u) != 0) {
                                const bool second = (uint32_t(bi.skip) & ((1u << r) - 1u)) != 0;
                                const uint32_t x0 = second ? x_second0 : x_first0, x1 = second ? x_second1 : x_first1;
                                z = min(z, min(x0 & 0xFFu, x1 & 0xFFu));
                                top = hrow_rgba8_packed(x0, x1, ax.fr);
                            }
                        }
                        const float2 w = wy[r];
                        out[r] = vmix_rgba8_weights(top, bot, w.x, w.y);
                        top = bot;
                        if (r + 1 == kRows) carry_z = z_row;
                    }
                } else {
                    H4p held = top;
                    uint32_t z_row = 1;
#pragma unroll
                    for (uint32_t r = 0; r < kRows; r++) {
                        arrived(r + 1, raw0[r + 1], raw1[r + 1]);
                        const bool again = r > 0 && ((uint32_t(bi.rep) >> r) & 1u) != 0;
                        H4p bot = top;
                        if (!again) {
                            z_row = min(raw0[r + 1] & 0xFFu, raw1[r + 1] & 0xFFu);
                            z = min(z, z_row);
                            bot = hrow_rgba8_packed(raw0[r + 1], raw1[r + 1], ax.fr);
                        }
                        const H4p upper = again ? held : top;
                        const float2 w = wy[r];
                        out[r] = vmix_rgba8_weights(upper, bot, w.x, w.y);
                        held = upper;
                        top = bot;
                        if (r + 1 == kRows) carry_z = z_row;
                    }
                }
                carry_top = top;
                carry_row = bi.y_last;
            } else {
                carry_row = -1;
            }
            bi = block_info(blk + 2u);
            request(bi, raw0, raw1, extra);
            if (__builtin_expect(chained, 1)) {
                if (__builtin_expect(__ballot(used && z == 0u) != 0ull, 0)) {
                    fast = false;
                } else if (used && !BT_ABLATE(A, 2u)) {
                    const global_wbytes_t rowq = tile_bytes + (b + cr0) * T * 4u;
#pragma unroll
                    for (uint32_t r = 0; r < kRows; r++)
                        asm volatile("global_store_dword %0, %1, %2" ::"v"(so[r]), "v"(out[r]), "s"(rowq) : "memory");
                }
            }
            if (__builtin_expect(!fast, 0)) {
                bool keep[kRows];
#pragma unroll
                for (uint32_t r = 0; r < kRows; r++) keep[r] = false;
#pragma unroll
                for (uint32_t r = 0; r < kRows; r++) {
                    if (r >= nrows) continue;
                    const Axis ay = ay_blk[r];
                    const global_u32_t row0 = (global_u32_t)(data + uint64_t(ay.i0) * raster.pitch), row1 = (global_u32_t)(data + uint64_t(ay.i1) * raster.pitch);
                    const H4 top = hrow_rgba8(row0[ax.i0], row0[ax.i1], ax.fr), bot = hrow_rgba8(row1[ax.i0], row1[ax.i1], ax.fr);
                    keep[r] = !(top.valid && bot.valid);
                    out[r] = vmix_rgba8(top, bot, ay.fr);
                }
                bool any_keep = false;
#pragma unroll
                for (uint32_t r = 0; r < kRows; r++) {
                    if (used && r < nrows && !keep[r]) tile[(b + cr0 + r) * T + store_px] = out[r];
                    any_keep = any_keep || keep[r];
                }
                if (__ballot(used && any_keep)) {
#pragma unroll
                    for (uint32_t r = 0; r < kRows; r++)
                        if (used && r < nrows && keep[r]) {
                            out[r] = A.prev_zero ? 0u : atlas[uint64_t(home) * tile_texels + (b + cr0 + r) * T + b + home_col];
                            if (apron_lane && !A.prev_zero) tile[(b + cr0 + r) * T + store_px] = out[r];
                        }
                }
#pragma unroll
                for (uint32_t r = 0; r < kRows; r++) asm volatile("" : "+v"(out[r]));
            }
            if (A.levels < 2 || self4 == kInvalid || BT_ABLATE(A, 1u)) return;
            uint32_t q[kRows / 2];
            uint32_t zr = 0xFFFFFFFFu;
#pragma unroll
            for (uint32_t r = 0; r < kRows; r++) zr = min(zr, out[r] << 8);
            if (__builtin_expect(nrows == kRows && !__ballot(active && zr == 0u), 1)) {
#pragma unroll
                for (uint32_t i = 0; i < kRows / 2; i++) {
                    const uint32_t l0 = quad_dpp<0xA0>(out[2 * i]), l1 = quad_dpp<0xA0>(out[2 * i + 1]);
                    const uint32_t r0 = quad_dpp<0xF5>(out[2 * i]), r1 = quad_dpp<0xF5>(out[2 * i + 1]);
                    const uint32_t mine = downsample4_rgba8_half(l0, l1, r0, r1, half_sh) << half_sh;
                    q[i] = mine | quad_dpp<0xB1>(mine);
                }
            } else {
#pragma unroll
                for (uint32_t i = 0; i < kRows / 2; i++) {
                    const uint32_t v = downsample4_rgba8(out[2 * i], out[2 * i + 1], quad_dpp<0xB1>(out[2 * i]), quad_dpp<0xB1>(out[2 * i + 1]));
                    q[i] = quad_dpp<0xA0>(v);
                }
            }
            {
                const global_wbytes_t row4 = base4 + (cr0 >> 1) * T * 4u;
                if (active && (tid & 1u) == 0) {
#pragma unroll
                    for (uint32_t i = 0; i < kRows / 2; i++)
                        if (2 * i + 1 < nrows) *(global_wu32_t)(row4 + i * T * 4u + l4) = q[i];
                }
            }
            if (A.levels < 3 || self3 == kInvalid) return;
            uint32_t w[kRows / 4];
            uint32_t zq = 0xFFFFFFFFu;
#pragma unroll
            for (uint32_t i = 0; i < kRows / 2; i++) zq = min(zq, q[i] << 8);
            if (__builtin_expect(nrows == kRows && !__ballot(active && zq == 0u), 1)) {
#pragma unroll
                for (uint32_t j = 0; j < kRows / 4; j++) {
                    const uint32_t l0 = quad_dpp<0x00>(q[2 * j]), l1 = quad_dpp<0x00>(q[2 * j + 1]);
                    const uint32_t r0 = quad_dpp<0xAA>(q[2 * j]), r1 = quad_dpp<0xAA>(q[2 * j + 1]);
                    const uint32_t mine = downsample4_rgba8_half(l0, l1, r0, r1, half_sh) << half_sh;
                    w[j] = mine | quad_dpp<0xB1>(mine);
                }
            } else {
#pragma unroll
                for (uint32_t j = 0; j < kRows / 4; j++)
                    w[j] = downsample4_rgba8(quad_dpp<0x00>(q[2 * j]), quad_dpp<0x00>(q[2 * j + 1]), quad_dpp<0xAA>(q[2 * j]), quad_dpp<0xAA>(q[2 * j + 1]));
            }
            {
                const global_wbytes_t row3 = base3 + (cr0 >> 2) * T * 4u;
#pragma unroll
                for (uint32_t j = 0; j < kRows / 4; j++)
                    if (active && (tid & 3u) == 0 && 4 * j + 3 < nrows) *(global_wu32_t)(row3 + j * T * 4u + l3) = w[j];
            }
        };
        if (BT_ABLATE(A, 16u)) continue;
        info_a = block_info(blk_begin);
        request(info_a, set_a0, set_a1, extra_a);
        info_b = block_info(blk_begin + 1u);
        request(info_b, set_b0, set_b1, extra_b);
        for (uint32_t blk = blk_begin;;) {
            block(blk, info_a, set_a0, set_a1, extra_a);
            if (++blk >= blk_end) break;
            block(blk, info_b, set_b0, set_b1, extra_b);
            if (++blk >= blk_end) break;
        }
        stamp(2u + cx0 / 256u);
    }

    const uint32_t n_cols = aprons_in_sweep ? 0u : (row_end - row_begin) * 2u * b;
    const uint32_t row_px = 2u * b * T, share = (row_px + wgs_per_tile - 1u) / wgs_per_tile;
    const uint32_t px_begin = min((work % wgs_per_tile) * share, row_px), px_end = min(px_begin + share, row_px);
    for (uint32_t i = tid; i < n_cols + (px_end - px_begin) && !BT_ABLATE(A, 4u); i += 256u) {
        uint32_t px, py;
        if (i < n_cols) {
            const uint32_t r = i / (2u * b), k = i % (2u * b);
            px = k < b ? k : c + k;
            py = b + row_begin + r;
        } else {
            const uint32_t e = px_begin + (i - n_cols), r = e / T;
            px = e % T;
            py = r < b ? r : c + r;
        }
        const int rx = px < b ? -1 : (px >= b + c ? 1 : 0), ry = py < b ? -1 : (py >= b + c ? 1 : 0);
        const uint32_t n = grid_lookup(A, it.side, A.lod, int(it.x) + rx, int(it.y) + ry);
        const bool have = n != kInvalid;
        const uint32_t sx = have ? uint32_t(int(it.x) + rx) : it.x, sy = have ? uint32_t(int(it.y) + ry) : it.y;
        const uint32_t qx = have ? uint32_t(int(px) - int(b) - rx * int(c)) : min(max(px, b), b + c - 1u) - b;
        const uint32_t qy = have ? uint32_t(int(py) - int(b) - ry * int(c)) : min(max(py, b), b + c - 1u) - b;
        tile[py * T + px] = rgba8_value_slow(A, raster, sx, qx, sy, qy, have ? n : it.atlas_index);
    }
    stamp(4);
}

__global__ void selftest_kernel(uint32_t* failures) {
    const uint32_t t = blockIdx.x * blockDim.x + threadIdx.x;
    if (t < 65536u) {
        volatile float d = 65535.0f;
        if (unorm16_to_float(t) != float(t) / d) atomicAdd(failures, 1u);
        const float x = float(t);
        if (__builtin_fmaf(x, 1.0f / 65535.0f, x) != 65536.0f * (x / d)) atomicAdd(failures, 1u);
    }
    if (t < 256u) {
        volatile float d = 255.0f;
        const float x = float(t), r = 1.0f / 255.0f, q0 = x * r;
        if (__builtin_fmaf(__builtin_fmaf(-q0, 255.0f, x), r, q0) != x / d) atomicAdd(failures, 1u);
        if (__builtin_fmaf(x, r, x) != 256.0f * (x / d)) atomicAdd(failures, 1u);
    }
}

}


struct FusedJobDev {
    FusedArgs args;
    uint32_t attachment;
    uint32_t queue_job = 0;
    uint32_t lds_pad = 0;
    std::vector<MainItem> host_items;
    uint32_t seam_first = 0;
    std::vector<uint32_t> finest_layers, all_layers;
};

struct FusedState {
    std::vector<FusedJobDev> jobs;
    void* arrays = nullptr;
    std::vector<uint8_t> whole_raster;
};

}

#include <algorithm>
namespace bt {

static FusedState& state_of(bt_preprocessor* p) {
    if (!p->fused) p->fused = new FusedState();
    return *p->fused;
}

void fused_release(bt_preprocessor* p) {
    if (!p->fused) return;
    hipFree(p->fused->arrays);
    delete p->fused;
    p->fused = nullptr;
}

struct JobGrid {
    uint32_t sides = 1, lod_lo = 0, lod_hi = 0;
    std::vector<uint32_t> offsets, cells;
    JobGrid() = default;
    JobGrid(uint32_t sides_, uint32_t lo, uint32_t hi) : sides(sides_), lod_lo(lo), lod_hi(hi), offsets(6 * 32, kInvalid) {
        for (uint32_t side = 0; side < sides; side++)
            for (uint32_t lod = lod_lo; lod <= lod_hi; lod++) {
                offsets[side * 32 + lod] = uint32_t(cells.size());
                cells.resize(cells.size() + (size_t(1) << (2 * lod)), kInvalid);
            }
    }
    bool holds(const bt_tile_coordinate& c) const { return c.side < sides && c.lod >= lod_lo && c.lod <= lod_hi && c.x < (1u << c.lod) && c.y < (1u << c.lod); }
    uint32_t& cell(const bt_tile_coordinate& c) { return cells[offsets[c.side * 32 + c.lod] + (size_t(c.x) << c.lod) + c.y]; }
    uint32_t cell(const bt_tile_coordinate& c) const { return cells[offsets[c.side * 32 + c.lod] + (size_t(c.x) << c.lod) + c.y]; }
    template <typename F>
    bool for_each(uint32_t lo, uint32_t end, F&& f) const {
        for (uint32_t side = 0; side < sides; side++)
            for (uint32_t lod = lo; lod < end; lod++) {
                const uint32_t* g = cells.data() + offsets[side * 32 + lod];
                for (uint32_t x = 0; x < (1u << lod); x++)
                    for (uint32_t y = 0; y < (1u << lod); y++)
                        if (!f(side, lod, x, y, g[(size_t(x) << lod) + y])) return false;
            }
        return true;
    }
    uint64_t tiles_at(uint32_t lod) const {
        uint64_t n = 0;
        for_each(lod, lod + 1, [&](uint32_t, uint32_t, uint32_t, uint32_t, uint32_t v) {
            n += v != kInvalid;
            return true;
        });
        return n;
    }
};

struct JobPlan {
    uint32_t job = 0;
    std::vector<const Task*> splits, downs, stitches;
    uint32_t ai = 0;
    AttachmentMeta m{};
    bool direct = false, hybrid = false;
    bool spherical = false;
    uint32_t main_levels = 1;
    JobGrid grid;
    bool shard = false;
    uint32_t strip_shift = 0, strips = 0, units_per_rank = 0;
    std::vector<MainItem> items;
    FusedArgs args{};
    uint64_t source_bytes = 0;
    std::vector<uint32_t> finest_layers, all_layers;

    uint32_t main_lo() const { return grid.lod_hi - (main_levels - 1); }
    bool rows_in_tail() const { return !shard && main_lo() > grid.lod_lo && main_levels > 1 && (direct || m.border_size % 2u == 0); }
    uint64_t tile_bytes() const { return uint64_t(m.texture_size) * m.texture_size * m.pixel_size; }
    uint64_t apron_bytes() const { return 2 * (2 * uint64_t(m.border_size) * (m.texture_size + m.center_size)) * m.pixel_size; }
    FusedJobDev fused_job() const {
        FusedJobDev d{args, ai};
        d.queue_job = job;
        return d;
    }
};

struct PlanOut {
    std::vector<TaskDev>& tasks;
    std::vector<Launch>& plan;
    FusedState& state;
};

static Launch job_launch(const JobPlan& j, LaunchKind kind, uint32_t variant) {
    Launch l{};
    l.kind = kind;
    l.variant = variant;
    l.attachment = j.ai;
    return l;
}

static bool collect_job(const bt_preprocessor* p, const bt_atlas* a, uint32_t job, JobPlan& j) {
    j.job = job;
    for (const Task& t : p->queue) {
        if (t.job != job) continue;
        if (t.type == kSplit) j.splits.push_back(&t);
        else if (t.type == kDownsample) j.downs.push_back(&t);
        else if (t.type == kStitch) j.stitches.push_back(&t);
    }
    if (j.splits.empty()) return false;
    j.ai = j.splits[0]->attachment_index;
    const AttachmentMeta& m = j.m = a->attachments[j.ai].meta;
    const bool tail_ok = (m.format == BT_FORMAT_R16 || m.format == BT_FORMAT_RGBA8) && (m.center_size & 3u) == 0 &&
                         m.center_size >= 2 * m.border_size && m.border_size != 0 && (m.format != BT_FORMAT_R16 || (m.border_size & 1u) == 0);
    const bool main_ok = tail_ok && m.format == BT_FORMAT_R16 && m.texture_size <= 512 && m.border_size <= 8;
    if (!tail_ok) return false;
    j.direct = !main_ok && m.format == BT_FORMAT_RGBA8;
    j.hybrid = !main_ok && !j.direct;
    const uint32_t lod_hi = j.splits[0]->coord.lod;
    uint32_t lod_lo = lod_hi;
    for (const Task* t : j.downs) lod_lo = std::min(lod_lo, t->coord.lod);
    if (lod_hi > 13) return false;
    j.spherical = a->config.spherical != 0;
    j.grid = JobGrid(j.spherical ? 6u : 1u, lod_lo, lod_hi);
    j.main_levels = j.hybrid ? 1u : std::min(3u, lod_hi - lod_lo + 1);
    return true;
}

static bool fill_grid(JobPlan& j) {
    JobGrid& g = j.grid;
    for (const Task* t : j.splits) {
        if (!g.holds(t->coord) || t->coord.lod != g.lod_hi) return false;
        g.cell(t->coord) = t->atlas_index;
    }
    for (const Task* t : j.downs) {
        if (!g.holds(t->coord)) return false;
        g.cell(t->coord) = t->atlas_index;
    }
    return true;
}

static bool qualifies(const JobPlan& j) {
    const JobGrid& g = j.grid;
    for (const Task* t : j.downs) {
        bt_tile_coordinate ch[4];
        tile_children(t->coord, ch);
        for (int k = 0; k < 4; k++)
            if (g.cell(ch[k]) == kInvalid) return false;
    }
    size_t present = 0;
    for (uint32_t v : g.cells) present += v != kInvalid;
    if (present != j.stitches.size()) return false;
    for (const Task* t : j.stitches) {
        const bt_tile_coordinate& c = t->coord;
        if (!g.holds(c) || g.cell(c) != t->atlas_index) return false;
        bt_tile_coordinate nb[8];
        tile_neighbours(c, false, nb);
        for (int i = 0; i < 8; i++) {
            const bool same_face = !is_invalid(nb[i]);
            const uint32_t in_grid = same_face ? g.cell(nb[i]) : kInvalid;
            const bool recorded_same_face = t->rel[i].atlas_index != BT_INVALID_ATLAS_INDEX && t->rel[i].coordinate.side == c.side && same_face;
            if (same_face && in_grid != (recorded_same_face ? t->rel[i].atlas_index : kInvalid)) return false;
        }
    }
    const Task* s0 = j.splits[0];
    for (const Task* t : j.splits)
        if (t->tl[0] != s0->tl[0] || t->tl[1] != s0->tl[1] || t->br[0] != s0->br[0] || t->br[1] != s0->br[1]) return false;
    return true;
}

static void plan_shards(bt_preprocessor* p, JobPlan& j) {
    const JobGrid& g = j.grid;
    const uint32_t world = p->shard_world, levels = std::min(3u, g.lod_hi - g.lod_lo + 1);
    j.strip_shift = levels - 1;
    j.strips = 1u << (g.lod_hi - j.strip_shift);
    const uint32_t units = g.sides * j.strips;
    j.shard = world > 1 && units % world == 0 && !j.hybrid;
    if (!j.shard) return;
    j.units_per_rank = units / world;
    auto base_of = [&](uint32_t side, uint32_t lod) { return g.cells[g.offsets[side * 32 + lod]]; };
    j.shard = g.for_each(g.lod_hi + 1 - levels, g.lod_hi + 1, [&](uint32_t side, uint32_t lod, uint32_t x, uint32_t y, uint32_t v) {
        const uint32_t base = base_of(side, lod);
        return base != kInvalid && v == base + ((x << lod) + y);
    });
    if (!j.shard) return;
    for (uint32_t side = 0; side < g.sides; side++)
        for (uint32_t k = 0; k < levels; k++) {
            const uint32_t lod = g.lod_hi - k, n = 1u << lod, base = base_of(side, lod), cols_per_strip = n / j.strips;
            for (uint32_t strip = 0; strip < j.strips;) {
                const uint32_t owner = (side * j.strips + strip) / j.units_per_rank;
                uint32_t end = strip + 1;
                while (end < j.strips && (side * j.strips + end) / j.units_per_rank == owner) end++;
                p->shard_pieces.push_back({j.ai, side, lod, base + strip * cols_per_strip * n, (end - strip) * cols_per_strip * n, owner});
                strip = end;
            }
            if (g.sides == 1) p->shard_ranges.push_back({j.ai, side, lod, base, n / world * n});
        }
}

static void order_items(const bt_preprocessor* p, JobPlan& j) {
    for (const Task* t : j.splits) {
        if (j.shard && (t->coord.side * j.strips + (t->coord.x >> j.strip_shift)) / j.units_per_rank != p->shard_rank) continue;
        j.items.push_back({t->coord.side, t->coord.x, t->coord.y, t->atlas_index, uint32_t(t->raster)});
    }
    std::stable_sort(j.items.begin(), j.items.end(), [](const MainItem& a, const MainItem& b2) {
        return a.side != b2.side ? a.side < b2.side : (a.y != b2.y ? a.y < b2.y : a.x < b2.x);
    });
}

static bool regular_layout(const JobGrid& g, uint32_t* first) {
    const uint32_t hi4 = 4u << (2u * g.lod_hi), per_side = (hi4 - (1u << (2u * g.lod_lo))) / 3u, f = g.cells.empty() ? 0u : g.cells[g.offsets[g.lod_hi]];
    *first = f;
    return f != kInvalid && g.for_each(g.lod_lo, g.lod_hi + 1, [&](uint32_t side, uint32_t lod, uint32_t x, uint32_t y, uint32_t v) {
        return v == f + side * per_side + (hi4 - (4u << (2u * lod))) / 3u + ((x << lod) + y);
    });
}

static void describe_job(const bt_preprocessor* p, const bt_atlas* a, JobPlan& j) {
    FusedArgs& args = j.args;
    args.m = j.m;
#ifdef BT_DEBUG_HOOKS
    if (const char* e = getenv("BT_FUSED_ABLATE")) args.ablate = uint32_t(strtoul(e, nullptr, 0));
#endif
    args.atlas = (uint16_t*)a->attachments[j.ai].level0;
    args.rasters = p->rasters_dev;
    args.tlx = j.splits[0]->tl[0];
    args.tly = j.splits[0]->tl[1];
    args.brx = j.splits[0]->br[0];
    args.bry = j.splits[0]->br[1];
    args.sides = j.grid.sides;
    args.grid_lod_lo = j.grid.lod_lo;
    args.grid_lod_hi = j.grid.lod_hi;
    args.grid_sides = j.grid.sides;
    args.regular = regular_layout(j.grid, &args.reg_first) ? 1u : 0u;
    std::vector<bool> seen(p->rasters.size(), false);
    for (const Task* t : j.splits)
        if (!seen[t->raster]) {
            seen[t->raster] = true;
            j.source_bytes += uint64_t(p->rasters[t->raster].dev.width) * p->rasters[t->raster].dev.height * j.m.pixel_size;
        }
    j.grid.for_each(j.grid.lod_lo, j.grid.lod_hi + 1, [&](uint32_t, uint32_t lod, uint32_t, uint32_t, uint32_t v) {
        if (v != kInvalid) {
            j.all_layers.push_back(v);
            if (lod == j.grid.lod_hi) j.finest_layers.push_back(v);
        }
        return true;
    });
}

static uint64_t main_bytes(const JobPlan& j) {
    uint64_t bytes = j.source_bytes;
    for (uint32_t k = 0; k < j.main_levels; k++) bytes += j.grid.tiles_at(j.grid.lod_hi - k) * j.tile_bytes();
    return bytes;
}

static FusedJobDev main_job(const JobPlan& j) {
    FusedJobDev job = j.fused_job();
    job.args.lod = j.grid.lod_hi;
    job.args.levels = j.main_levels;
    job.args.item_count = uint32_t(j.items.size());
    job.host_items = j.items;
    job.finest_layers = j.finest_layers;
    job.all_layers = j.all_layers;
    return job;
}

static void plan_hybrid(const JobPlan& j, PlanOut& out) {
    Launch ls = job_launch(j, kLaunchSplit, BT_VARIANT_HYBRID);
    ls.first_task = uint32_t(out.tasks.size());
    for (const Task* t : j.splits) {
        out.tasks.push_back(to_device_task(*t));
        if (t->raster >= 0 && size_t(t->raster) < out.state.whole_raster.size()) out.state.whole_raster[size_t(t->raster)] = 1;
    }
    ls.task_count = uint32_t(j.splits.size());
    ls.algorithmic_bytes = j.source_bytes + uint64_t(j.splits.size()) * j.tile_bytes();
    out.plan.push_back(ls);
    Launch lt = job_launch(j, kLaunchStitch, BT_VARIANT_HYBRID);
    lt.first_task = uint32_t(out.tasks.size());
    for (const Task* t : j.stitches)
        if (t->coord.lod == j.grid.lod_hi) out.tasks.push_back(to_device_task(*t));
    lt.task_count = uint32_t(out.tasks.size()) - lt.first_task;
    lt.algorithmic_bytes = uint64_t(lt.task_count) * j.apron_bytes();
    if (lt.task_count) out.plan.push_back(lt);
}

static void plan_direct(const bt_preprocessor* p, const JobPlan& j, PlanOut& out) {
    FusedJobDev job = main_job(j);
    bool rep = false, skips = false;
    {
        const double mosaic = double(j.m.center_size) * double(1u << j.grid.lod_hi);
        for (const Task* t : j.splits) {
            const RasterDev& r = p->rasters[t->raster].dev;
            const double ratio = double(r.height) / (double(j.args.bry - j.args.tly) * mosaic);
            if (ratio < 0.9999) rep = true;
            if (ratio > 1.02) skips = true;
        }
    }
    {
        const uint64_t blocks = uint64_t(j.items.size()) * ((j.m.center_size + kDirectRows - 1) / kDirectRows);
        job.args.groups = uint32_t(std::min<uint64_t>(kDirectMaxBlocks, std::max<uint64_t>(1, (blocks + 1023) / 1024)));
#ifdef BT_DEBUG_HOOKS
        if (const char* e = getenv("BT_FUSED_PARTS")) job.args.groups = std::max(1u, std::min(kDirectMaxBlocks, uint32_t(atoi(e))));
#endif
    }
    Launch ld = job_launch(j, kLaunchFusedDirect, rep ? BT_VARIANT_DIRECT_REP : skips ? BT_VARIANT_DIRECT_SKIPS : BT_VARIANT_DIRECT);
    ld.task_count = uint32_t(j.items.size());
    ld.aux0 = uint32_t(out.state.jobs.size());
    ld.algorithmic_bytes = main_bytes(j);
    out.state.jobs.push_back(job);
    out.plan.push_back(ld);
}

static uint32_t size_main_window(const bt_preprocessor* p, const JobPlan& j, FusedArgs& A) {
    const AttachmentMeta& m = j.m;
    const uint32_t lod_hi = j.grid.lod_hi;
    double ratio_x = 0.0, ratio_y = 0.0;
    uint64_t max_pitch = 0;
    bool aligned = true;
    const double mosaic = double(1u << lod_hi) * double(m.center_size);
    for (const Task* t : j.splits) {
        const RasterDev& r = p->rasters[t->raster].dev;
        max_pitch = std::max<uint64_t>(max_pitch, r.pitch);
        ratio_x = std::max(ratio_x, double(r.width) / (double(A.brx - A.tlx) * mosaic));
        ratio_y = std::max(ratio_y, double(r.height) / (double(A.bry - A.tly) * mosaic));
        if (((reinterpret_cast<uintptr_t>(r.data) | r.pitch) & 15u) != 0) aligned = false;
    }
    const uint32_t rows = std::min(kMainRows, m.center_size) + 2 * m.border_size;
    const uint64_t cols_needed = uint64_t(double(m.texture_size - 1) * ratio_x) + 4 + 7;
    uint64_t rows_needed = uint64_t(double(rows - 1) * ratio_y) + 4;
    uint64_t exact_core = rows_needed;
    {
        const uint32_t c = m.center_size, b = m.border_size, chunks = (c + kMainRows - 1) / kMainRows;
        const float scale = float(1u << lod_hi);
        uint64_t exact = 1;
        exact_core = 1;
        std::vector<std::pair<uint32_t, int>> seen;
        for (const Task* t : j.splits) {
            const std::pair<uint32_t, int> key(t->coord.y, t->raster);
            if (std::find(seen.begin(), seen.end(), key) != seen.end()) continue;
            seen.push_back(key);
            const uint32_t H = p->rasters[t->raster].dev.height, n = 1u << lod_hi, ty = t->coord.y;
            auto axis = [&](uint32_t tile, uint32_t r) { return split_axis(r, c, tile, scale, A.tly, A.bry, H); };
            for (uint32_t k = 0; k < chunks; k++) {
                const uint32_t r0 = k * kMainRows, r1 = std::min(c, r0 + kMainRows) - 1;
                int lo = axis(ty, r0).i0, hi = axis(ty, r1).i1;
                exact_core = std::max<uint64_t>(exact_core, uint64_t(hi - lo + 1));
                if (k == 0) lo = std::min(lo, ty > 0 ? axis(ty - 1, c - b).i0 : axis(ty, 0).i0);
                if (k == chunks - 1) hi = std::max(hi, ty + 1 < n ? axis(ty + 1, b - 1).i1 : axis(ty, c - 1).i1);
                exact = std::max<uint64_t>(exact, uint64_t(hi - lo + 1));
            }
        }
        rows_needed = std::min(rows_needed, exact);
    }
    const uint64_t pitch = (cols_needed + 7) / 8 * 8;
    const uint64_t budget = 65536 - sizeof(MainShared);
    A.lds_pitch = uint32_t(std::min<uint64_t>(pitch, 1u << 20));
    const uint64_t kQuarter = (160u << 10) / 4, kThird = (160u << 10) / 3, fixed = sizeof(MainShared);
    const uint64_t core_rows = std::min(rows_needed, exact_core);
    const bool dma_variant = aligned && pitch <= 4096 && pitch != 528 && (m.texture_size == 512 || core_rows * (pitch / 8) > 256 * 4);
    {
        const uint64_t with_aprons = fixed + 2 * rows_needed * pitch * 2, core = fixed + 2 * core_rows * pitch * 2;
        auto groups = [&](uint64_t bytes) { return bytes <= kQuarter ? 4 : bytes <= kThird ? 3 : bytes <= (80u << 10) ? 2 : 1; };
        if (dma_variant && groups(core) > groups(with_aprons)) {
            A.apron_global = 1;
            rows_needed = core_rows;
        }
    }
    uint64_t buffers = 2;
    if (dma_variant && fixed + 2 * rows_needed * pitch * 2 > kQuarter && fixed + core_rows * pitch * 2 <= kQuarter) {
        A.single_buffer = 1;
        A.apron_global = 1;
        rows_needed = core_rows;
        buffers = 1;
    }
    const bool fits_lds = buffers * rows_needed * pitch * 2 <= budget && (rows_needed + 1) * max_pitch < (1ull << 31);
    const bool fits_batch = rows_needed * (pitch / 8) <= 256 * 4;
    const bool dma_only = fits_lds && aligned && pitch <= 4096 && (!fits_batch || m.texture_size == 512);
    A.lds_rows = fits_lds && (fits_batch || dma_only) ? uint32_t(rows_needed) : 0u;
    if ((A.apron_global || A.single_buffer) && A.lds_rows && !dma_only) {
        A.apron_global = 0;
        A.single_buffer = 0;
        A.lds_rows = 0;
    }
    if (!A.lds_rows) return BT_VARIANT_MAIN_UNSTAGED;
    if (aligned && m.texture_size == 512 && A.lds_pitch == 528) return BT_VARIANT_MAIN_DMA_528;
    if (dma_only) return A.single_buffer ? BT_VARIANT_MAIN_SINGLE_BUFFER : A.apron_global ? BT_VARIANT_MAIN_APRON_GLOBAL : BT_VARIANT_MAIN_DMA_PITCH;
    return BT_VARIANT_MAIN_REG_PITCH;
}

static void plan_main(const bt_preprocessor* p, const JobPlan& j, PlanOut& out) {
    FusedJobDev job = main_job(j);
#ifdef BT_DEBUG_HOOKS
    if (const char* e = getenv("BT_FUSED_LDS_PAD")) job.lds_pad = uint32_t(atoi(e));
#endif
    {
        const uint32_t chunks = (j.m.center_size + kMainRows - 1) / kMainRows;
        uint32_t parts = 1;
#ifdef BT_DEBUG_HOOKS
        if (const char* e = getenv("BT_FUSED_PARTS")) parts = uint32_t(atoi(e));
        else
#endif
        {
            while (parts < chunks && uint64_t(j.items.size()) * parts < 1024) parts++;
            for (uint32_t cand = parts; cand <= std::min(chunks, parts + 8); cand++)
                if ((uint64_t(j.items.size()) * cand) % 1024 == 0) { parts = cand; break; }
        }
        parts = std::max(parts, (chunks + kMaxChunks - 1) / kMaxChunks);
        job.args.groups = std::max(1u, std::min(parts, chunks));
    }
    Launch lm = job_launch(j, kLaunchFusedMain, size_main_window(p, j, job.args));
    job.args.rotate_priority = 1;
    lm.kernels = lm.variant == BT_VARIANT_MAIN_UNSTAGED ? 2u : 1u;
    lm.task_count = uint32_t(j.items.size());
    lm.aux0 = uint32_t(out.state.jobs.size());
    lm.algorithmic_bytes = main_bytes(j);
    out.state.jobs.push_back(job);
    out.plan.push_back(lm);
}

static void plan_apron_stitch(const JobPlan& j, PlanOut& out) {
    if (j.main_levels <= 1 || j.rows_in_tail()) return;
    Launch ls = job_launch(j, kLaunchStitch, BT_VARIANT_STITCH_LAUNCH);
    ls.first_task = uint32_t(out.tasks.size());
    for (const Task* t : j.stitches)
        if (t->coord.lod != j.grid.lod_hi && t->coord.lod + j.main_levels > j.grid.lod_hi) out.tasks.push_back(to_device_task(*t));
    ls.task_count = uint32_t(out.tasks.size()) - ls.first_task;
    ls.algorithmic_bytes = uint64_t(ls.task_count) * j.apron_bytes();
    ls.phase = j.shard ? 2u : 0u;
    ls.aux0 = (j.shard || j.direct) ? 0u : 1u;
    if (!j.shard && !j.direct) ls.algorithmic_bytes = uint64_t(ls.task_count) * 2 * (2 * j.m.border_size * uint64_t(j.m.texture_size)) * j.m.pixel_size;
    if (ls.task_count) out.plan.push_back(ls);
}

struct TailPlan {
    int job = -1, plan = -1;
    uint32_t launches = 0;
};

static TailPlan plan_tails(const JobPlan& j, PlanOut& out) {
    const uint64_t Tt = j.m.texture_size, cc = j.m.center_size, bpp = j.m.pixel_size;
    TailPlan tails;
    for (uint32_t in_lod = j.main_lo(); in_lod > j.grid.lod_lo;) {
        tails.launches++;
        const uint32_t levels = std::min(3u, in_lod - j.grid.lod_lo);
        FusedJobDev tail = j.fused_job();
        tail.all_layers = j.all_layers;
        tail.args.lod = in_lod;
        tail.args.levels = levels;
        tail.args.apron_lods = (j.rows_in_tail() && in_lod == j.main_lo()) ? j.main_levels - 1 : 0u;
        tail.args.apron_cols = j.direct ? 1u : 0u;
        Launch lt = job_launch(j, kLaunchFusedTail, j.args.regular ? BT_VARIANT_TAIL_REGULAR : BT_VARIANT_TAIL_IRREGULAR);
        lt.aux0 = uint32_t(out.state.jobs.size());
        lt.phase = j.shard ? 2u : 0u;
        lt.algorithmic_bytes = j.grid.tiles_at(in_lod) * cc * cc * bpp;
        for (uint32_t k = 0; k < tail.args.apron_lods; k++) lt.algorithmic_bytes += j.grid.tiles_at(in_lod + k) * 2 * (2 * j.m.border_size * (Tt + (j.direct ? cc : 0))) * bpp;
        for (uint32_t k = 1; k <= levels; k++) {
            lt.algorithmic_bytes += j.grid.tiles_at(in_lod - k) * j.tile_bytes();
            lt.task_count += uint32_t(j.grid.tiles_at(in_lod - k));
        }
        if (tails.job < 0) {
            tails.job = int(out.state.jobs.size());
            tails.plan = int(out.plan.size());
        }
        out.state.jobs.push_back(tail);
        out.plan.push_back(lt);
        in_lod -= levels;
    }
    return tails;
}

static bool seams_covered(const JobPlan& j, uint32_t lo, uint32_t end, bool pulled) {
    std::unordered_set<uint32_t> stitched;
    for (const Task* t : j.stitches) {
        if (!on_face_edge(t->coord) || t->coord.lod < lo || t->coord.lod >= end) continue;
        stitched.insert(t->atlas_index);
        const int n = int(1u << t->coord.lod);
        for (int i = 0; i < 8; i++) {
            const int nx = int(t->coord.x) + kNeighbourOffsets[i][0], ny = int(t->coord.y) + kNeighbourOffsets[i][1];
            const bool out_x = nx < 0 || nx >= n, out_y = ny < 0 || ny >= n;
            const bt_atlas_tile& r = t->rel[i];
            const bool across = r.atlas_index != BT_INVALID_ATLAS_INDEX && r.coordinate.side != t->coord.side;
            if (out_x != out_y && !(across && (!pulled || (r.coordinate.lod == t->coord.lod && r.coordinate.x < 65536u && r.coordinate.y < 65536u))))
                return false;
        }
    }
    return j.grid.for_each(lo, end, [&](uint32_t, uint32_t lod, uint32_t x, uint32_t y, uint32_t v) {
        return !(on_face_edge({0, lod, x, y}) && v != kInvalid && !stitched.count(v));
    });
}

static void plan_cube_seams(const JobPlan& j, const TailPlan& tails, PlanOut& out) {
    const AttachmentMeta& m = j.m;
    const uint32_t main_lo = j.main_lo(), lod_hi = j.grid.lod_hi;
    const bool in_tail = !j.shard && !j.hybrid && tails.job >= 0 && out.state.jobs[size_t(tails.job)].args.apron_lods != 0 &&
                         seams_covered(j, main_lo, lod_hi, false);
    const bool pull = in_tail && tails.launches == 1 && seams_covered(j, j.grid.lod_lo, main_lo, true);
    uint64_t tail_pixels = 0, late_pixels = 0;
    const uint32_t tail_first = uint32_t(out.tasks.size());
    for (int pass = 0; pass < 2; pass++) {
        if (pass == 1 && in_tail) {
            FusedJobDev& tj = out.state.jobs[size_t(tails.job)];
            tj.seam_first = tail_first;
            tj.args.seam_count = uint32_t(out.tasks.size()) - tail_first;
            tj.args.seam_skip = 1;
            tj.args.seam_pull = pull ? 1u : 0u;
            out.plan[size_t(tails.plan)].algorithmic_bytes += 2 * tail_pixels * m.pixel_size;
        }
        const uint32_t first = uint32_t(out.tasks.size());
        for (int sweep = (pass == 0 && pull) ? 0 : 1; sweep < 2; sweep++)
            for (const Task* t : j.stitches) {
                if (!on_face_edge(t->coord)) continue;
                if (j.hybrid && t->coord.lod == lod_hi) continue;
                const bool pulled = pull && t->coord.lod < main_lo;
                const bool rides = in_tail && (t->coord.lod >= main_lo || pulled);
                if (rides != (pass == 0)) continue;
                if (pass == 0 && pull && pulled != (sweep == 0)) continue;
                const TaskDev d = to_device_task(*t);
                for (int i = 0; i < 8; i++)
                    if (d.rel_index[i] != BT_INVALID_ATLAS_INDEX && d.rel_side[i] != d.side) {
                        TaskDev e = d;
                        e.regions = 1u << i;
                        uint32_t parts = 1;
                        if (pulled) {
                            const uint32_t pixels = m.border_size * (i < 4 ? m.center_size : m.border_size);
                            const uint32_t pairs = (m.format != BT_FORMAT_R16 || ((m.border_size | m.texture_size) & 1u)) ? pixels : pixels / 2u;
                            parts = std::max(1u, std::min(255u, (pairs + 255u) / 256u));
                            e.rel_index[i] = (t->rel[i].coordinate.x << 16) | t->rel[i].coordinate.y;
                        }
                        for (uint32_t part = 0; part < parts; part++) {
                            if (pulled) e.raster = (main_lo - t->coord.lod) | (part << 8) | (parts << 16);
                            out.tasks.push_back(e);
                        }
                        (pass == 0 ? tail_pixels : late_pixels) += uint64_t(m.border_size) * (i < 4 ? m.center_size : m.border_size);
                    }
            }
        if (pass == 0) continue;
        Launch ls = job_launch(j, kLaunchStitch, BT_VARIANT_STITCH_LAUNCH);
        ls.aux0 = 2u;
        ls.first_task = first;
        ls.task_count = uint32_t(out.tasks.size()) - first;
        ls.algorithmic_bytes = 2 * late_pixels * m.pixel_size;
        ls.phase = j.shard ? 2u : 0u;
        if (ls.task_count) out.plan.push_back(ls);
    }
}

static bt_status fused_upload(FusedState& state, const std::vector<std::vector<MainItem>>& items, const std::vector<std::vector<uint32_t>>& grids) {
    std::vector<size_t> at(2 * items.size());
    size_t bytes = 0;
    for (size_t k = 0; k < at.size(); k++) {
        at[k] = (bytes + 255) & ~size_t(255);
        bytes = at[k] + (k % 2 ? grids[k / 2].size() * sizeof(uint32_t) : items[k / 2].size() * sizeof(MainItem));
    }
    BT_HIP(hipMalloc(&state.arrays, bytes ? bytes : 1));
    uint8_t* base = (uint8_t*)state.arrays;
    for (size_t k = 0; k < items.size(); k++) {
        if (!items[k].empty()) BT_HIP(hipMemcpy(base + at[2 * k], items[k].data(), items[k].size() * sizeof(MainItem), hipMemcpyHostToDevice));
        if (!grids[k].empty()) BT_HIP(hipMemcpy(base + at[2 * k + 1], grids[k].data(), grids[k].size() * sizeof(uint32_t), hipMemcpyHostToDevice));
    }
    for (FusedJobDev& job : state.jobs) {
        job.args.items = (const MainItem*)(base + at[2 * job.queue_job]);
        job.args.grids = (const uint32_t*)(base + at[2 * job.queue_job + 1]);
    }
    return BT_OK;
}

bool fused_plan(bt_preprocessor* p, bt_atlas* a, std::vector<TaskDev>& tasks, std::vector<Launch>& plan) {
    FusedState& state = state_of(p);
    hipFree(state.arrays);
    state.arrays = nullptr;
    state.jobs.clear();
    state.whole_raster.assign(p->rasters.size(), 0);
    if (p->queue.empty()) return false;

    PlanOut out{tasks, plan, state};
    std::vector<std::vector<MainItem>> items;
    std::vector<std::vector<uint32_t>> grids;
    for (uint32_t job = 0; job < p->jobs; job++) {
        JobPlan j;
        if (!collect_job(p, a, job, j) || !fill_grid(j) || !qualifies(j)) return false;
        plan_shards(p, j);
        order_items(p, j);
        describe_job(p, a, j);
        if (j.hybrid) plan_hybrid(j, out);
        else if (j.direct) plan_direct(p, j, out);
        else plan_main(p, j, out);
        plan_apron_stitch(j, out);
        const TailPlan tails = plan_tails(j, out);
        if (j.spherical) plan_cube_seams(j, tails, out);
        items.push_back(std::move(j.items));
        grids.push_back(std::move(j.grid.cells));
    }
    return fused_upload(state, items, grids) == BT_OK;
}

uint32_t fused_begin_run(bt_preprocessor* p, bt_atlas* a) {
    uint32_t flagged = 0;
    for (const Launch& l : p->plan) {
        Attachment& at = a->attachments[l.attachment];
        if (l.kind == kLaunchSplit || l.kind == kLaunchDownsample || l.kind == kLaunchStitch) {
            for (uint32_t i = l.first_task; i < l.first_task + l.task_count && i < p->tasks_host.size(); i++) at.mark_written(p->tasks_host[i].atlas_index, 1);
            continue;
        }
        if (!p->fused || l.aux0 >= p->fused->jobs.size()) continue;
        FusedJobDev& job = p->fused->jobs[l.aux0];
        if (l.kind == kLaunchFusedMain || l.kind == kLaunchFusedDirect) {
            bool fresh = !job.finest_layers.empty();
            for (uint32_t layer : job.finest_layers) fresh = fresh && layer < at.written.size() && !at.written[layer];
            job.args.prev_zero = fresh ? 1u : 0u;
            flagged += fresh;
        }
        for (uint32_t layer : job.all_layers) at.mark_written(layer, 1);
    }
    return flagged;
}

bool fused_source_window(const bt_preprocessor* p, uint32_t raster, uint32_t out[4]) {
    if (!p->fused || raster >= p->rasters.size()) return false;
    if (raster < p->fused->whole_raster.size() && p->fused->whole_raster[raster]) return false;
    const RasterDev& r = p->rasters[raster].dev;
    uint32_t x0 = r.width, y0 = r.height, x1 = 0, y1 = 0;
    bool any = false, known = false;
    for (const Launch& l : p->plan) {
        if ((l.kind != kLaunchFusedMain && l.kind != kLaunchFusedDirect) || l.aux0 >= p->fused->jobs.size()) continue;
        const FusedJobDev& job = p->fused->jobs[l.aux0];
        if (job.host_items.empty()) continue;
        known = true;
        const bool direct = l.variant == BT_VARIANT_DIRECT || l.variant == BT_VARIANT_DIRECT_REP || l.variant == BT_VARIANT_DIRECT_SKIPS;
        const FusedArgs& A = job.args;
        const uint32_t c = A.m.center_size, b = A.m.border_size, n = 1u << A.lod;
        const float scale = float(n);
        auto ax = [&](uint32_t tile, uint32_t col) { return split_axis(col, c, tile, scale, A.tlx, A.brx, r.width); };
        auto ay = [&](uint32_t tile, uint32_t row) { return split_axis(row, c, tile, scale, A.tly, A.bry, r.height); };
        for (const MainItem& it : job.host_items) {
            if (it.raster != raster) continue;
            any = true;
            const int lo_x = std::min(it.x > 0 ? ax(it.x - 1, c - b).i0 : ax(it.x, 0).i0, ax(it.x, 0).i0);
            const int hi_x = std::max(it.x + 1 < n ? ax(it.x + 1, b - 1).i1 : ax(it.x, c - 1).i1, ax(it.x, c - 1).i1);
            const int lo_y = std::min(it.y > 0 ? ay(it.y - 1, c - b).i0 : ay(it.y, 0).i0, ay(it.y, 0).i0);
            const int hi_y = std::max(it.y + 1 < n ? ay(it.y + 1, b - 1).i1 : ay(it.y, c - 1).i1, ay(it.y, c - 1).i1);
            uint32_t xa = uint32_t(std::max(lo_x, 0)), xe = uint32_t(hi_x) + 1u;
            if (!direct) {
                xa &= ~7u;
                if (l.variant != BT_VARIANT_MAIN_UNSTAGED) xe = std::max(xe, xa + A.lds_pitch);
                if (xe + 8u > r.width) xe = r.width;
            }
            x0 = std::min(x0, xa);
            x1 = std::max(x1, std::min(xe, r.width));
            y0 = std::min(y0, uint32_t(std::max(lo_y, 0)));
            y1 = std::max(y1, std::min(uint32_t(hi_y) + 1u, r.height));
        }
    }
    if (!known) return false;
    if (!any) x0 = y0 = x1 = y1 = 0;
    out[0] = x0;
    out[1] = y0;
    out[2] = x1;
    out[3] = y1;
    return true;
}

bool fused_stream_bands(bt_preprocessor* p, const Launch& l, uint32_t tile_rows_per_band, std::vector<StreamBand>* bands) {
    if ((l.kind != kLaunchFusedMain && l.kind != kLaunchFusedDirect) || !p->fused || l.aux0 >= p->fused->jobs.size()) return false;
    const FusedJobDev& job = p->fused->jobs[l.aux0];
    const std::vector<MainItem>& items = job.host_items;
    if (items.empty() || l.variant == BT_VARIANT_MAIN_UNSTAGED) return false;
    const uint32_t c = job.args.m.center_size, b = job.args.m.border_size, n = 1u << job.args.lod;
    if (tile_rows_per_band == 0) tile_rows_per_band = std::max(1u, std::min(4u, n / 4u));
    const float scale = float(n);
    bands->clear();
    size_t i = 0;
    while (i < items.size()) {
        const uint32_t side = items[i].side, raster = items[i].raster;
        if (raster >= p->rasters.size()) return false;
        const RasterDev& r = p->rasters[raster].dev;
        auto axis = [&](uint32_t tile, uint32_t row) { return split_axis(row, c, tile, scale, job.args.tly, job.args.bry, r.height); };
        StreamBand band{};
        band.item_begin = uint32_t(i);
        band.tile_y_begin = items[i].y;
        band.side = side;
        band.raster = raster;
        uint32_t rows = 0, y = items[i].y;
        while (i < items.size() && items[i].side == side && (items[i].y == y || rows + 1 < tile_rows_per_band)) {
            if (items[i].raster != raster) return false;
            if (items[i].y != y) {
                if (items[i].y < y) return false;
                y = items[i].y;
                rows++;
            }
            i++;
        }
        band.item_count = uint32_t(i) - band.item_begin;
        band.tile_y_end = y + 1;
        const int hi = y + 1 < n ? axis(y + 1, b - 1).i1 : axis(y, c - 1).i1;
        band.source_row_end = uint32_t(std::min<int64_t>(int64_t(r.height), int64_t(hi) + 1));
        if (!bands->empty() && bands->back().raster == raster) {
            if (bands->back().source_row_end > band.source_row_end) return false;
        } else {
            for (const StreamBand& earlier : *bands)
                if (earlier.raster == raster) return false;
        }
        bands->push_back(band);
    }
    return true;
}

void fused_launch_tiles(const bt_preprocessor* p, const Launch& l, uint32_t item_begin, uint32_t item_count, std::vector<FusedTile>* out) {
    out->clear();
    if ((l.kind != kLaunchFusedMain && l.kind != kLaunchFusedDirect) || !p->fused || l.aux0 >= p->fused->jobs.size()) return;
    const FusedJobDev& job = p->fused->jobs[l.aux0];
    for (uint64_t i = item_begin; i < uint64_t(item_begin) + item_count && i < job.host_items.size(); i++) {
        const MainItem& it = job.host_items[size_t(i)];
        out->push_back({{it.side, job.args.lod, it.x, it.y}, it.atlas_index});
    }
}

bt_status fused_launch_range(bt_preprocessor* p, bt_atlas* a, const Launch& l, uint32_t item_begin, uint32_t item_count) {
    (void)a;
    if (!p->fused || l.aux0 >= p->fused->jobs.size()) {
        set_error("fused launch without a plan");
        return BT_ERR_INVALID_ARGUMENT;
    }
    FusedJobDev job = p->fused->jobs[l.aux0];
    FusedArgs& A = job.args;
    A.rasters = p->rasters_dev;
    if ((l.kind == kLaunchFusedMain || l.kind == kLaunchFusedDirect) && item_begin < A.item_count) {
        A.items += item_begin;
        A.item_count = std::min(item_count, A.item_count - item_begin);
    }
    const hipStream_t stream = p->ctx->stream;
    auto direct_blocks = [&] {
        const uint32_t blocks_per_tile = (A.m.center_size + kDirectRows - 1) / kDirectRows;
        return A.item_count * ((blocks_per_tile + A.groups - 1) / A.groups);
    };
    const uint32_t main_blocks = A.item_count * A.groups;
    const size_t main_lds = std::min<size_t>(65536, sizeof(MainShared) + (A.single_buffer ? 1 : 2) * size_t(A.lds_rows) * A.lds_pitch * 2 + job.lds_pad);
    switch (l.variant) {
        case BT_VARIANT_DIRECT:
            fused_direct_rgba8_kernel<false><<<direct_blocks(), 256, 0, stream>>>(A);
            break;
        case BT_VARIANT_DIRECT_REP:
            fused_direct_rgba8_kernel<true><<<direct_blocks(), 256, 0, stream>>>(A);
            break;
        case BT_VARIANT_DIRECT_SKIPS:
            fused_direct_rgba8_kernel<false, true><<<direct_blocks(), 256, 0, stream>>>(A);
            break;
        case BT_VARIANT_MAIN_DMA_528:
            fused_main_kernel<true, false, 512, 528, true><<<main_blocks, 256, main_lds, stream>>>(A);
            break;
        case BT_VARIANT_MAIN_DMA_PITCH:
        case BT_VARIANT_MAIN_APRON_GLOBAL:
        case BT_VARIANT_MAIN_SINGLE_BUFFER:
            fused_main_kernel<true, false, 0, 0, true><<<main_blocks, 256, main_lds, stream>>>(A);
            break;
        case BT_VARIANT_MAIN_REG_PITCH:
            fused_main_kernel<true, false, 0, 0><<<main_blocks, 256, main_lds, stream>>>(A);
            break;
        case BT_VARIANT_MAIN_UNSTAGED:
            fused_corner_kernel<<<A.item_count, 64, 0, stream>>>(A);
            fused_main_kernel<false, true, 0, 0><<<main_blocks, 256, sizeof(MainShared), stream>>>(A);
            break;
        case BT_VARIANT_TAIL_REGULAR:
        case BT_VARIANT_TAIL_IRREGULAR: {
            const uint32_t size = (1u << A.lod) * A.m.center_size, nx = (size + 63) / 64;
            A.seam_tasks = p->tasks_dev + job.seam_first;
            uint64_t extras = 0;
            if (A.apron_lods) {
                const uint32_t blocks_per_tile = A.m.format == BT_FORMAT_R16
                    ? (A.m.border_size * A.m.texture_size + 256u * kApronPairsPerThread - 1u) / (256u * kApronPairsPerThread)
                    : (2u * A.m.border_size * (A.m.texture_size + (A.apron_cols ? A.m.center_size : 0u)) + 255u) / 256u;
                for (uint32_t k = 0; k < A.apron_lods; k++) extras += (1ull << (2 * (A.lod + k))) * blocks_per_tile;
            }
            A.tail_extras = uint32_t(extras);
            const uint64_t total_m = uint64_t(A.sides) * nx * nx, total_a = uint64_t(A.sides) * extras;
            const uint32_t blocks = uint32_t(8 * ((total_m + 7) / 8 + (total_a + 7) / 8 + (uint64_t(A.seam_count) + 7) / 8));
            const bool regular = l.variant == BT_VARIANT_TAIL_REGULAR;
            if (A.m.format == BT_FORMAT_R16) {
                if (regular) fused_tail_kernel<BT_FORMAT_R16, true><<<blocks, 256, 0, stream>>>(A);
                else fused_tail_kernel<BT_FORMAT_R16, false><<<blocks, 256, 0, stream>>>(A);
            } else {
                if (regular) fused_tail_kernel<BT_FORMAT_RGBA8, true><<<blocks, 256, 0, stream>>>(A);
                else fused_tail_kernel<BT_FORMAT_RGBA8, false><<<blocks, 256, 0, stream>>>(A);
            }
            break;
        }
        default:
            set_error("fused launch of variant 0x%x", l.variant);
            return BT_ERR_INVALID_ARGUMENT;
    }
    hipError_t e = hipGetLastError();
    if (e != hipSuccess) return hip_fail(e, "fused kernel launch");
    return BT_OK;
}

}

extern "C" bt_status bt_selftest(bt_ctx* ctx, uint32_t* failures) {
    if (!ctx || !failures) return BT_ERR_INVALID_ARGUMENT;
    BT_HIP(hipSetDevice(ctx->device));
    uint32_t* dev = nullptr;
    BT_HIP(hipMalloc((void**)&dev, sizeof(uint32_t)));
    hipError_t e = hipMemsetAsync(dev, 0, sizeof(uint32_t), ctx->stream);
    if (e == hipSuccess) {
        bt::selftest_kernel<<<256, 256, 0, ctx->stream>>>(dev);
        e = hipGetLastError();
    }
    if (e == hipSuccess) e = hipMemcpyAsync(failures, dev, sizeof(uint32_t), hipMemcpyDeviceToHost, ctx->stream);
    if (e == hipSuccess) e = hipStreamSynchronize(ctx->stream);
    hipFree(dev);
    if (e != hipSuccess) return bt::hip_fail(e, "bt_selftest");
    return BT_OK;
}
```

Measured before the change: 4.684 million tiles/s.

## Precompute per-tile neighbour records and row tables on host for the main kernel

Builds per-item MainRecord structs (neighbour indices, parent tiles, x-window start, apron extensions) and shared per-(raster,row) row/window tables at plan time and uploads them. The main kernel no longer does grid lookups, per-row split_axis setup or the two __syncthreads window reductions. It loads the tables into LDS with 16-byte vector loads overlapped with the first DMA/stage issue and the corner texel fetches. This trades extra plan-time host work and device memory for a shorter kernel prologue with fewer barriers.

```diff
diff --git a/bevy_terrain_amd/csrc/bt_fused.hip b/bevy_terrain_amd/csrc/bt_fused.hip
--- a/bevy_terrain_amd/csrc/bt_fused.hip
+++ b/bevy_terrain_amd/csrc/bt_fused.hip
@@ -29,11 +29,38 @@
     uint32_t side, x, y, atlas_index, raster;
 };
 
+struct alignas(16) MainRecord {
+    uint32_t side, x, y, self;
+    uint32_t raster, n, e, s;
+    uint32_t w, nw, ne, se;
+    uint32_t sw, self4, self3, table;
+    uint32_t x4l, x4r, x3l, x3r;
+    uint32_t xa;
+    uint32_t ext_lo, ext_hi;
+    uint32_t pad;
+};
+struct MainStart {
+    int ymin;
+    uint32_t slots;
+};
+struct TableLayout {
+    uint32_t fy, ymin, slots, bytes;
+};
+__host__ __device__ __forceinline__ TableLayout table_layout(uint32_t chunks) {
+    const uint32_t win = (chunks * 4u + 15u) & ~15u;
+    return {chunks * 32u, chunks * 96u, chunks * 96u + win, chunks * 96u + 2u * win};
+}
+constexpr uint32_t kRasterRuns = 6;
+
 struct FusedArgs {
     AttachmentMeta m;
     uint16_t* atlas;
     const RasterDev* rasters;
     const MainItem* items;
+    const MainRecord* records;
+    const MainStart* starts;
+    const uint8_t* tables;
+    uint32_t run_end[kRasterRuns - 1], run_raster[kRasterRuns];
     const uint32_t* grids;
     uint32_t grid_lod_lo, grid_lod_hi, grid_sides;
     uint32_t regular, reg_first;
@@ -108,17 +135,6 @@
 struct TileNb {
     uint32_t self, n, e, s, w;
 };
-
-__device__ __forceinline__ TileNb load_tile_nb(const FusedArgs& A, uint32_t side, uint32_t lod, uint32_t x, uint32_t y) {
-    const int ix = int(x), iy = int(y);
-    TileNb t;
-    t.self = grid_lookup(A, side, lod, ix, iy);
-    t.n = grid_lookup(A, side, lod, ix, iy - 1);
-    t.e = grid_lookup(A, side, lod, ix + 1, iy);
-    t.s = grid_lookup(A, side, lod, ix, iy + 1);
-    t.w = grid_lookup(A, side, lod, ix - 1, iy);
-    return t;
-}
 
 template <bool kCentre = true, typename TT = uint16_t>
 __device__ __forceinline__ void push_pixel(const FusedArgs& A, uint32_t side, uint32_t lod, uint32_t tx, uint32_t ty,
@@ -280,24 +296,34 @@
     return out;
 }
 
-__device__ __forceinline__ uint32_t split_value_slow(const FusedArgs& A, const RasterDev& r, uint32_t tx, uint32_t rx, uint32_t ty,
-                                                  uint32_t ry, uint32_t home_index) {
+struct SlowTexels {
+    uint32_t t00, t10, t01, t11;
+    float fx, fy;
+};
+__device__ __forceinline__ SlowTexels split_texels_slow(const FusedArgs& A, const RasterDev& r, uint32_t tx, uint32_t rx, uint32_t ty, uint32_t ry) {
     const float scale = float(1u << A.lod);
-    const uint32_t c = A.m.center_size, b = A.m.border_size, T = A.m.texture_size;
+    const uint32_t c = A.m.center_size;
     const Axis ax = split_axis(rx, c, tx, scale, A.tlx, A.brx, r.width);
     const Axis ay = split_axis(ry, c, ty, scale, A.tly, A.bry, r.height);
     typedef const uint8_t __attribute__((address_space(1))) * global_bytes;
     typedef const uint16_t __attribute__((address_space(1))) * global_u16;
     const global_u16 row0 = (global_u16)((global_bytes)r.data + uint64_t(ay.i0) * r.pitch);
     const global_u16 row1 = (global_u16)((global_bytes)r.data + uint64_t(ay.i1) * r.pitch);
-    const uint32_t t00 = row0[ax.i0], t10 = row0[ax.i1], t01 = row1[ax.i0], t11 = row1[ax.i1];
-    if (t00 == 0 || t10 == 0 || t01 == 0 || t11 == 0) {
+    return {row0[ax.i0], row0[ax.i1], row1[ax.i0], row1[ax.i1], ax.fr, ay.fr};
+}
+__device__ __forceinline__ uint32_t split_finish_slow(const FusedArgs& A, const SlowTexels& s, uint32_t rx, uint32_t ry, uint32_t home_index) {
+    const uint32_t b = A.m.border_size, T = A.m.texture_size;
+    if (s.t00 == 0 || s.t10 == 0 || s.t01 == 0 || s.t11 == 0) {
         if (home_index == kInvalid || A.prev_zero) return 0;
         return A.atlas[uint64_t(home_index) * T * T + uint64_t(b + ry) * T + b + rx];
     }
-    const float top = mixf(unorm16_to_float(t00), unorm16_to_float(t10), ax.fr);
-    const float bot = mixf(unorm16_to_float(t01), unorm16_to_float(t11), ax.fr);
-    return float_to_unorm16(mixf(top, bot, ay.fr));
+    const float top = mixf(unorm16_to_float(s.t00), unorm16_to_float(s.t10), s.fx);
+    const float bot = mixf(unorm16_to_float(s.t01), unorm16_to_float(s.t11), s.fx);
+    return float_to_unorm16(mixf(top, bot, s.fy));
+}
+__device__ __forceinline__ uint32_t split_value_slow(const FusedArgs& A, const RasterDev& r, uint32_t tx, uint32_t rx, uint32_t ty,
+                                                  uint32_t ry, uint32_t home_index) {
+    return split_finish_slow(A, split_texels_slow(A, r, tx, rx, ty, ry), rx, ry, home_index);
 }
 
 __device__ __forceinline__ uint32_t xcd_remap(uint32_t bid, uint32_t total) {
@@ -329,10 +355,10 @@
     int win_ymin[kMaxChunks];
     uint32_t win_slots[kMaxChunks];
     RowParam apron[2 * kMaxBorder];
-    int xmin, xmax;
-    uint32_t pad_[2];
+    uint32_t pad_[4];
 };
 static_assert(sizeof(MainShared) % 16 == 0, "LDS carve must stay 16-byte aligned");
+static_assert(offsetof(MainShared, row_fy) % 16 == 0 && offsetof(MainShared, win_ymin) % 16 == 0 && offsetof(MainShared, win_slots) % 16 == 0, "the row table arrives in 16-byte pieces");
 
 struct Texel4 {
     float a0, a1, b0, b1;
@@ -370,15 +396,22 @@
 }
 
 template <bool kStaged, bool kGeneric, uint32_t kT, uint32_t kP, bool kDma = false>
-__device__ __forceinline__ void fused_main_chunks(const FusedArgs& A, uint32_t item_index, uint32_t k_begin, uint32_t k_end, uint8_t* smem) {
+__device__ __forceinline__ void fused_main_chunks(const FusedArgs& A, uint32_t item_index, uint32_t part, uint32_t k_begin, uint32_t k_end, uint8_t* smem) {
     MainShared& S = *reinterpret_cast<MainShared*>(smem);
     uint16_t* s_buf = reinterpret_cast<uint16_t*>(smem + sizeof(MainShared));
     constexpr bool kFix = kStaged && !kGeneric;
     const bool one_buffer = kDma && kP == 0 && A.single_buffer != 0;
     const uint32_t buf_texels = one_buffer ? 0u : A.lds_rows * (kP ? kP : A.lds_pitch);
 
-    const MainItem it = A.items[item_index];
-    const RasterDev raster = A.rasters[it.raster];
+    const MainRecord rec = A.records[item_index];
+    const MainStart start = A.starts[item_index * A.groups + part];
+    uint32_t raster_hint = A.run_raster[0];
+#pragma unroll
+    for (uint32_t i = 0; i + 1 < kRasterRuns; i++)
+        if (item_index >= A.run_end[i]) raster_hint = A.run_raster[i + 1];
+    RasterDev raster = A.rasters[raster_hint];
+    if (rec.raster != raster_hint) raster = A.rasters[rec.raster];
+    const MainItem it{rec.side, rec.x, rec.y, rec.self, rec.raster};
     const uint32_t T = kT ? kT : A.m.texture_size, b = A.m.border_size, c = A.m.center_size, o = b + c;
     const uint32_t tid = threadIdx.x;
 #ifdef BT_DEBUG_HOOKS
@@ -394,76 +427,10 @@
     const uint32_t tile_texels = T * T;
     const uint32_t chunks_per_tile = (c + kMainRows - 1) / kMainRows;
 
-    const TileNb t5 = load_tile_nb(A, it.side, A.lod, it.x, it.y);
-    const uint32_t self4 = A.levels >= 2 ? grid_lookup(A, it.side, A.lod - 1, int(it.x >> 1), int(it.y >> 1)) : kInvalid;
-    const uint32_t self3 = A.levels >= 3 ? grid_lookup(A, it.side, A.lod - 2, int(it.x >> 2), int(it.y >> 2)) : kInvalid;
-
-    for (uint32_t i = tid; i < (k_end - k_begin) * kMainRows; i += 256u) {
-        const uint32_t cr = k_begin * kMainRows + i;
-        if (cr < c) {
-            const Axis ay = split_axis(cr, c, it.y, scale, A.tly, A.bry, raster.height);
-            S.row_y0[i] = ay.i0 | (ay.i1 == ay.i0 ? int(0x80000000u) : 0);
-            S.row_fy[i] = float2{ay.fr, 1.0f - ay.fr};
-        }
-    }
-    if (tid >= 32 && tid < 32 + 2 * b) {
-        const uint32_t r = tid - 32, k = r % b;
-        const bool top = r < b;
-        const uint32_t nrow = top ? t5.n : t5.s;
-        uint32_t ty, ry;
-        if (nrow != kInvalid) { ty = top ? it.y - 1 : it.y + 1; ry = top ? c - b + k : k; } else { ty = it.y; ry = top ? 0u : c - 1; }
-        const Axis ay = split_axis(ry, c, ty, scale, A.tly, A.bry, raster.height);
-        S.apron[r].y0 = ay.i0;
-        S.apron[r].y1 = ay.i1;
-        S.apron[r].fy = ay.fr;
-        S.apron[r].pad = ry;
-    }
-
-    const uint32_t half_c = c / 2, half_b = b / 2;
-    const bool is_centre = tid < half_c;
-    const bool is_right = !is_centre && tid < half_c + half_b;
-    const bool is_left = !is_centre && !is_right && tid < half_c + 2 * half_b;
-    const bool is_idle = !is_centre && !is_right && !is_left;
-    uint32_t px0 = 0;
-    uint32_t txa = it.x, txb = it.x, rxa = 0, rxb = 0;
-    if (is_centre) {
-        px0 = b + 2 * tid;
-        rxa = 2 * tid;
-        rxb = 2 * tid + 1;
-    } else if (is_right) {
-        const uint32_t j = 2 * (tid - half_c);
-        px0 = o + j;
-        if (t5.e != kInvalid) { txa = txb = it.x + 1; rxa = j; rxb = j + 1; } else { rxa = rxb = c - 1; }
-    } else if (is_left) {
-        const uint32_t j = 2 * (tid - half_c - half_b);
-        px0 = j;
-        if (t5.w != kInvalid) { txa = txb = it.x - 1; rxa = c - b + j; rxb = c - b + j + 1; } else { rxa = rxb = 0; }
-    }
-    const Axis axa = split_axis(rxa, c, txa, scale, A.tlx, A.brx, raster.width);
-    const Axis axb = split_axis(rxb, c, txb, scale, A.tlx, A.brx, raster.width);
-    const float fxa = axa.fr, fxb = axb.fr, gxa = 1.0f - fxa, gxb = 1.0f - fxb;
-    const uint32_t home_col = is_right && t5.e != kInvalid ? t5.e : (is_left && t5.w != kInvalid ? t5.w : t5.self);
-
-    if (tid == half_c + half_b) S.xmin = min(axa.i0, axb.i0);
-    if (tid == half_c + half_b - 1) S.xmax = max(axa.i1, axb.i1);
-    __syncthreads();
-    if (tid < k_end - k_begin) {
-        const uint32_t k = k_begin + tid, n = min(kMainRows, c - k * kMainRows);
-        const int* y0 = S.row_y0 + tid * kMainRows;
-        const int first = y0[0] & 0x7fffffff;
-        bool consecutive = n == kMainRows;
-        for (uint32_t i = 0; i < n; i++) consecutive = consecutive && y0[i] == first + int(i);
-        int lo = first, hi = (y0[n - 1] & 0x7fffffff) + (y0[n - 1] < 0 ? 0 : 1);
-        if (!(kDma && kP == 0 && A.apron_global)) {
-            if (k == 0) lo = min(lo, S.apron[0].y0);
-            if (k == chunks_per_tile - 1) hi = max(hi, S.apron[2 * b - 1].y1);
-        }
-        S.win_ymin[tid] = lo;
-        S.win_slots[tid] = uint32_t(hi - lo + 1) | (consecutive ? 0x80000000u : 0u);
-    }
-    __syncthreads();
-
-    const int xa = __builtin_amdgcn_readfirstlane(S.xmin) & ~7;
+    const TileNb t5{rec.self, rec.n, rec.e, rec.s, rec.w};
+    const uint32_t self4 = rec.self4, self3 = rec.self3;
+
+    const int xa = int(rec.xa);
     const uint32_t P = kP ? kP : A.lds_pitch;
     typedef const uint8_t __attribute__((address_space(1))) * global_bytes;
     typedef const uint16_t __attribute__((address_space(1))) * global_u16;
@@ -478,8 +445,8 @@
 
     auto chunk_rows = [&](uint32_t k) -> uint32_t { return min(kMainRows, c - k * kMainRows); };
     auto window = [&](uint32_t k, int& ymin, uint32_t& slots) {
-        ymin = __builtin_amdgcn_readfirstlane(S.win_ymin[k - k_begin]);
-        slots = uint32_t(__builtin_amdgcn_readfirstlane(S.win_slots[k - k_begin])) & 0x7fffffffu;
+        ymin = __builtin_amdgcn_readfirstlane(S.win_ymin[k]);
+        slots = (uint32_t(__builtin_amdgcn_readfirstlane(S.win_slots[k])) & 0x7fffffffu) + (k == chunks_per_tile - 1 ? rec.ext_hi : 0u);
     };
     uint32_t src_off[kBatch], lds_off[kBatch];
 #pragma unroll
@@ -545,6 +512,104 @@
         }
     };
 
+    int ymin = start.ymin;
+    uint32_t slots = start.slots;
+    u32x4 pre[kBatch];
+    if constexpr (kDma) {
+        dma_issue(s_buf + (k_begin & 1u) * buf_texels, ymin, slots);
+    } else if (kStaged && !BT_ABLATE(A, 8u)) {
+        if (wide) stage_issue(ymin, slots, pre);
+    }
+    constexpr uint32_t kTablePieces = (kMaxChunks * (kMainRows * 12u + 8u) / 16u + 255u) / 256u;
+    static_assert(kTablePieces == 2, "a whole table (kMaxChunks chunks) in two pieces per thread");
+    u32x4 table_piece[kTablePieces];
+    uint32_t table_dst[kTablePieces];
+    {
+        const TableLayout tl = table_layout(chunks_per_tile);
+        const global_bytes table = (global_bytes)A.tables + uint64_t(rec.table) * tl.bytes;
+        const uint32_t run = k_end - k_begin, p_y0 = 2u * run, p_fy = 4u * run, p_win = (tl.slots - tl.ymin) / 16u;
+#pragma unroll
+        for (uint32_t i = 0; i < kTablePieces; i++) {
+            const uint32_t p = tid + 256u * i;
+            uint32_t src = 0;
+            table_dst[i] = kInvalid;
+            if (p < p_y0) {
+                src = (2u * k_begin + p) * 16u;
+                table_dst[i] = uint32_t(offsetof(MainShared, row_y0)) + p * 16u;
+            } else if (p < p_y0 + p_fy) {
+                src = tl.fy + (4u * k_begin + p - p_y0) * 16u;
+                table_dst[i] = uint32_t(offsetof(MainShared, row_fy)) + (p - p_y0) * 16u;
+            } else if (p < p_y0 + p_fy + p_win) {
+                src = tl.ymin + (p - p_y0 - p_fy) * 16u;
+                table_dst[i] = uint32_t(offsetof(MainShared, win_ymin)) + (p - p_y0 - p_fy) * 16u;
+            } else if (p < p_y0 + p_fy + 2u * p_win) {
+                src = tl.slots + (p - p_y0 - p_fy - p_win) * 16u;
+                table_dst[i] = uint32_t(offsetof(MainShared, win_slots)) + (p - p_y0 - p_fy - p_win) * 16u;
+            }
+            table_piece[i] = *(global_u4)(table + src);
+        }
+    }
+    const bool has_corner = kStaged && k_begin == 0 && tid < 4u * b * b;
+    SlowTexels corner_texels{};
+    uint32_t corner_rx = 0, corner_ry = 0, corner_home = kInvalid, corner_dst = 0;
+    if (has_corner) {
+        const uint32_t corner = tid / (b * b), i = (tid % (b * b)) % b, j = (tid % (b * b)) / b;
+        const bool left = corner == 0 || corner == 3, top = corner < 2;
+        const uint32_t n = corner == 0 ? rec.nw : corner == 1 ? rec.ne : corner == 2 ? rec.se : rec.sw;
+        uint32_t tx = it.x, ty = it.y;
+        if (n != kInvalid) {
+            tx = left ? it.x - 1 : it.x + 1;
+            ty = top ? it.y - 1 : it.y + 1;
+            corner_rx = left ? c - b + i : i;
+            corner_ry = top ? c - b + j : j;
+            corner_home = n;
+        } else {
+            corner_rx = left ? 0u : c - 1;
+            corner_ry = top ? 0u : c - 1;
+            corner_home = t5.self;
+        }
+        corner_dst = (top ? j : o + j) * T + (left ? i : o + i);
+        corner_texels = split_texels_slow(A, raster, tx, corner_rx, ty, corner_ry);
+    }
+
+    if (tid >= 32 && tid < 32 + 2 * b) {
+        const uint32_t r = tid - 32, k = r % b;
+        const bool top = r < b;
+        const uint32_t nrow = top ? t5.n : t5.s;
+        uint32_t ty, ry;
+        if (nrow != kInvalid) { ty = top ? it.y - 1 : it.y + 1; ry = top ? c - b + k : k; } else { ty = it.y; ry = top ? 0u : c - 1; }
+        const Axis ay = split_axis(ry, c, ty, scale, A.tly, A.bry, raster.height);
+        S.apron[r].y0 = ay.i0;
+        S.apron[r].y1 = ay.i1;
+        S.apron[r].fy = ay.fr;
+        S.apron[r].pad = ry;
+    }
+
+    const uint32_t half_c = c / 2, half_b = b / 2;
+    const bool is_centre = tid < half_c;
+    const bool is_right = !is_centre && tid < half_c + half_b;
+    const bool is_left = !is_centre && !is_right && tid < half_c + 2 * half_b;
+    const bool is_idle = !is_centre && !is_right && !is_left;
+    uint32_t px0 = 0;
+    uint32_t txa = it.x, txb = it.x, rxa = 0, rxb = 0;
+    if (is_centre) {
+        px0 = b + 2 * tid;
+        rxa = 2 * tid;
+        rxb = 2 * tid + 1;
+    } else if (is_right) {
+        const uint32_t j = 2 * (tid - half_c);
+        px0 = o + j;
+        if (t5.e != kInvalid) { txa = txb = it.x + 1; rxa = j; rxb = j + 1; } else { rxa = rxb = c - 1; }
+    } else if (is_left) {
+        const uint32_t j = 2 * (tid - half_c - half_b);
+        px0 = j;
+        if (t5.w != kInvalid) { txa = txb = it.x - 1; rxa = c - b + j; rxb = c - b + j + 1; } else { rxa = rxb = 0; }
+    }
+    const Axis axa = split_axis(rxa, c, txa, scale, A.tlx, A.brx, raster.width);
+    const Axis axb = split_axis(rxb, c, txb, scale, A.tlx, A.brx, raster.width);
+    const float fxa = axa.fr, fxb = axb.fr, gxa = 1.0f - fxa, gxb = 1.0f - fxb;
+    const uint32_t home_col = is_right && t5.e != kInvalid ? t5.e : (is_left && t5.w != kInvalid ? t5.w : t5.self);
+
     uint16_t* tile5 = A.atlas + uint64_t(t5.self) * tile_texels;
     uint32_t* tile5_u32 = reinterpret_cast<uint32_t*>(tile5);
     uint16_t* tile4 = A.atlas + uint64_t(self4 == kInvalid ? 0u : self4) * tile_texels;
@@ -552,14 +617,14 @@
     const uint32_t cx4 = (it.x & 1u) * half_c + tid, cy4_base = (it.y & 1u) * half_c;
     const uint32_t cx3 = (it.x & 3u) * (c / 4) + (tid >> 1), cy3_base = (it.y & 3u) * (c / 4);
     const bool do4 = A.levels >= 2 && !BT_ABLATE(A, 1u), do3 = A.levels >= 3 && !BT_ABLATE(A, 1u);
-    auto make_xpush = [&](uint32_t shift, uint32_t self, uint32_t cx, uint32_t& layer, uint32_t& off, uint32_t& count) {
+    auto make_xpush = [&](uint32_t self, uint32_t nl, uint32_t nr, uint32_t cx, uint32_t& layer, uint32_t& off, uint32_t& count) {
         layer = 0;
         off = 0;
         count = 0;
         if (!is_centre || self == kInvalid) return;
         const bool left = cx < b, right = cx >= c - b;
         if (!left && !right) return;
-        const uint32_t n = grid_lookup(A, it.side, A.lod - shift, int(it.x >> shift) + (left ? -1 : 1), int(it.y >> shift));
+        const uint32_t n = left ? nl : nr;
         const uint32_t j = left ? cx : cx - (c - b);
         if (n != kInvalid) {
             layer = n;
@@ -572,8 +637,8 @@
         }
     };
     uint32_t x4_layer, x4_off, x4_count, x3_layer, x3_off, x3_count;
-    make_xpush(1, A.levels >= 2 ? self4 : kInvalid, cx4, x4_layer, x4_off, x4_count);
-    make_xpush(2, A.levels >= 3 ? self3 : kInvalid, cx3, x3_layer, x3_off, x3_count);
+    make_xpush(self4, rec.x4l, rec.x4r, cx4, x4_layer, x4_off, x4_count);
+    make_xpush(self3, rec.x3l, rec.x3r, cx3, x3_layer, x3_off, x3_count);
     auto xpush4 = [&](uint32_t cy, uint16_t v) {
         for (uint32_t e = 0; e < x4_count; e++) A.atlas[uint64_t(x4_layer) * tile_texels + x4_off + cy * T + e] = v;
     };
@@ -582,23 +647,13 @@
     };
     const uint32_t la0 = uint32_t(axa.i0 - xa), la1 = uint32_t(axa.i1 - xa), lb0 = uint32_t(axb.i0 - xa), lb1 = uint32_t(axb.i1 - xa);
 
-    int ymin = 0;
-    uint32_t slots = 0;
-    u32x4 pre[kBatch];
-    window(k_begin, ymin, slots);
-    if constexpr (kDma) {
-        dma_issue(s_buf + (k_begin & 1u) * buf_texels, ymin, slots);
-    } else if (kStaged && !BT_ABLATE(A, 8u)) {
-        if (wide) {
-            stage_issue(ymin, slots, pre);
-            stage_commit(s_buf + (k_begin & 1u) * buf_texels, slots, pre);
-        } else {
-            stage_narrow(s_buf + (k_begin & 1u) * buf_texels, ymin, slots);
-        }
-    }
-    if constexpr (kStaged) {
-        if (k_begin == 0) corner_pixels(A, item_index, tid, 256u);
-    }
+    if (kStaged && !kDma && !BT_ABLATE(A, 8u)) {
+        if (wide) stage_commit(s_buf + (k_begin & 1u) * buf_texels, slots, pre);
+        else stage_narrow(s_buf + (k_begin & 1u) * buf_texels, ymin, slots);
+    }
+#pragma unroll
+    for (uint32_t i = 0; i < kTablePieces; i++)
+        if (table_dst[i] != kInvalid) *reinterpret_cast<u32x4*>(smem + table_dst[i]) = table_piece[i];
     auto chunk_barrier = [&]() {
         if constexpr (kDma) asm volatile("s_waitcnt vmcnt(0)" ::: "memory");
         __syncthreads();
@@ -716,6 +771,7 @@
 
     chunk_barrier();
     wg_stamp(1);
+    if (has_corner) tile5[corner_dst] = uint16_t(split_finish_slow(A, corner_texels, corner_rx, corner_ry, corner_home));
 
     for (uint32_t k = k_begin; k < k_end; k++) {
         const int* row_y0 = S.row_y0 + (k - k_begin) * kMainRows;
@@ -768,7 +824,7 @@
                 auto quantise = [&](f2 v) -> f2 { return khalf + kn * v; };
                 auto quantise_quarter = [&](f2 s) -> f2 { return khalf + knq * s; };
                 const uint32_t cy4_first = cy4_base + (cr0 >> 1), cy3_first = cy3_base + (cr0 >> 2);
-                if (kMainRows == 8 && __builtin_amdgcn_readfirstlane(int(S.win_slots[k - k_begin])) < 0) {
+                if (kMainRows == 8 && __builtin_amdgcn_readfirstlane(int(S.win_slots[k])) < 0) {
                     const uint16_t* base = s_src + uint32_t(__builtin_amdgcn_readfirstlane(row_y0[0]) - cur_ymin) * P;
                     const uint16_t *pa0 = base + la0, *pa1 = base + la1, *pb0 = base + lb0, *pb1 = base + lb1;
                     const float2* fyt = row_fy;
@@ -1053,7 +1109,7 @@
 #include "bt_fused_debug.inc"
 #undef BT_FUSED_DEBUG_ENTRY_PRIORITY
 #endif
-    fused_main_chunks<kStaged, kGeneric, kT, kP, kDma>(A, work / A.groups, k_begin, k_end, smem);
+    fused_main_chunks<kStaged, kGeneric, kT, kP, kDma>(A, work / A.groups, part, k_begin, k_end, smem);
 }
 
 __global__ __launch_bounds__(64) void fused_corner_kernel(FusedArgs A) { corner_pixels(A, blockIdx.x, threadIdx.x, blockDim.x); }
@@ -1926,6 +1982,9 @@
     std::vector<MainItem> host_items;
     uint32_t seam_first = 0;
     std::vector<uint32_t> finest_layers, all_layers;
+    std::vector<MainRecord> records;
+    std::vector<MainStart> starts;
+    std::vector<uint8_t> tables;
 };
 
 struct FusedState {
@@ -2315,6 +2374,122 @@
     return BT_VARIANT_MAIN_REG_PITCH;
 }
 
+static void raster_runs(const std::vector<MainItem>& items, size_t begin, size_t count, FusedArgs& A) {
+    for (uint32_t k = 0; k + 1 < kRasterRuns; k++) A.run_end[k] = kInvalid;
+    for (uint32_t k = 0; k < kRasterRuns; k++) A.run_raster[k] = 0;
+    const size_t end = std::min(items.size(), begin + count);
+    uint32_t run = 0;
+    for (size_t i = begin; i < end; i++) {
+        if (i == begin) A.run_raster[0] = items[i].raster;
+        else if (items[i].raster != A.run_raster[run]) {
+            if (run + 1 == kRasterRuns) break;
+            A.run_end[run++] = uint32_t(i - begin);
+            A.run_raster[run] = items[i].raster;
+        }
+    }
+}
+
+static void build_main_records(const bt_preprocessor* p, const JobPlan& j, uint32_t variant, FusedJobDev& job) {
+    const FusedArgs& A = job.args;
+    const JobGrid& g = j.grid;
+    const uint32_t c = A.m.center_size, b = A.m.border_size, lod = A.lod, chunks = (c + kMainRows - 1) / kMainRows, groups = A.groups;
+    const float scale = float(1u << lod);
+    auto at = [&](uint32_t side, int l, int x, int y) -> uint32_t {
+        if (l < int(g.lod_lo) || l > int(g.lod_hi) || side >= g.sides) return kInvalid;
+        const int n = int(1u << l);
+        if (x < 0 || y < 0 || x >= n || y >= n) return kInvalid;
+        return g.cell(bt_tile_coordinate{side, uint32_t(l), uint32_t(x), uint32_t(y)});
+    };
+    const bool dma_pitch = variant == BT_VARIANT_MAIN_DMA_PITCH || variant == BT_VARIANT_MAIN_APRON_GLOBAL || variant == BT_VARIANT_MAIN_SINGLE_BUFFER;
+    const bool extend = !(dma_pitch && A.apron_global);
+    const TableLayout tl = table_layout(chunks);
+    std::vector<std::pair<uint32_t, uint32_t>> keys;
+    auto table_of = [&](uint32_t raster, uint32_t ty) -> uint32_t {
+        const std::pair<uint32_t, uint32_t> key(raster, ty);
+        for (size_t k = keys.size(); k-- > 0;)
+            if (keys[k] == key) return uint32_t(k);
+        keys.push_back(key);
+        job.tables.resize(keys.size() * size_t(tl.bytes), 0);
+        uint8_t* t = job.tables.data() + (keys.size() - 1) * size_t(tl.bytes);
+        int* row_y0 = reinterpret_cast<int*>(t);
+        float* row_fy = reinterpret_cast<float*>(t + tl.fy);
+        int* win_ymin = reinterpret_cast<int*>(t + tl.ymin);
+        uint32_t* win_slots = reinterpret_cast<uint32_t*>(t + tl.slots);
+        const uint32_t H = p->rasters[raster].dev.height;
+        for (uint32_t cr = 0; cr < c; cr++) {
+            const Axis ay = split_axis(cr, c, ty, scale, A.tly, A.bry, H);
+            row_y0[cr] = ay.i0 | (ay.i1 == ay.i0 ? int(0x80000000u) : 0);
+            row_fy[2 * cr] = ay.fr;
+            row_fy[2 * cr + 1] = 1.0f - ay.fr;
+        }
+        for (uint32_t k = 0; k < chunks; k++) {
+            const uint32_t n = std::min(kMainRows, c - k * kMainRows);
+            const int* y0 = row_y0 + k * kMainRows;
+            const int first = y0[0] & 0x7fffffff;
+            bool consecutive = n == kMainRows;
+            for (uint32_t i = 0; i < n; i++) consecutive = consecutive && y0[i] == first + int(i);
+            const int hi = (y0[n - 1] & 0x7fffffff) + (y0[n - 1] < 0 ? 0 : 1);
+            win_ymin[k] = first;
+            win_slots[k] = uint32_t(hi - first + 1) | (consecutive ? 0x80000000u : 0u);
+        }
+        return uint32_t(keys.size() - 1);
+    };
+    job.records.reserve(j.items.size());
+    job.starts.reserve(j.items.size() * size_t(groups));
+    for (const MainItem& it : j.items) {
+        const int x = int(it.x), y = int(it.y), l = int(lod);
+        const RasterDev& r = p->rasters[it.raster].dev;
+        MainRecord rec{};
+        rec.side = it.side;
+        rec.x = it.x;
+        rec.y = it.y;
+        rec.self = at(it.side, l, x, y);
+        rec.raster = it.raster;
+        rec.n = at(it.side, l, x, y - 1);
+        rec.e = at(it.side, l, x + 1, y);
+        rec.s = at(it.side, l, x, y + 1);
+        rec.w = at(it.side, l, x - 1, y);
+        rec.nw = at(it.side, l, x - 1, y - 1);
+        rec.ne = at(it.side, l, x + 1, y - 1);
+        rec.se = at(it.side, l, x + 1, y + 1);
+        rec.sw = at(it.side, l, x - 1, y + 1);
+        rec.self4 = A.levels >= 2 ? at(it.side, l - 1, x >> 1, y >> 1) : kInvalid;
+        rec.self3 = A.levels >= 3 ? at(it.side, l - 2, x >> 2, y >> 2) : kInvalid;
+        rec.x4l = A.levels >= 2 ? at(it.side, l - 1, (x >> 1) - 1, y >> 1) : kInvalid;
+        rec.x4r = A.levels >= 2 ? at(it.side, l - 1, (x >> 1) + 1, y >> 1) : kInvalid;
+        rec.x3l = A.levels >= 3 ? at(it.side, l - 2, (x >> 2) - 1, y >> 2) : kInvalid;
+        rec.x3r = A.levels >= 3 ? at(it.side, l - 2, (x >> 2) + 1, y >> 2) : kInvalid;
+        rec.table = table_of(it.raster, it.y);
+        {
+            const bool west = rec.w != kInvalid;
+            const Axis a0 = split_axis(west ? c - b : 0u, c, west ? it.x - 1 : it.x, scale, A.tlx, A.brx, r.width);
+            const Axis a1 = split_axis(west ? c - b + 1 : 0u, c, west ? it.x - 1 : it.x, scale, A.tlx, A.brx, r.width);
+            rec.xa = uint32_t(std::min(a0.i0, a1.i0)) & ~7u;
+        }
+        const uint8_t* t = job.tables.data() + size_t(rec.table) * tl.bytes;
+        const int* win_ymin = reinterpret_cast<const int*>(t + tl.ymin);
+        const uint32_t* win_slots = reinterpret_cast<const uint32_t*>(t + tl.slots);
+        if (extend) {
+            const Axis top = rec.n != kInvalid ? split_axis(c - b, c, it.y - 1, scale, A.tly, A.bry, r.height) : split_axis(0u, c, it.y, scale, A.tly, A.bry, r.height);
+            const Axis bottom = rec.s != kInvalid ? split_axis(b - 1, c, it.y + 1, scale, A.tly, A.bry, r.height) : split_axis(c - 1, c, it.y, scale, A.tly, A.bry, r.height);
+            const int lo = win_ymin[0], hi = win_ymin[chunks - 1] + int(win_slots[chunks - 1] & 0x7fffffffu) - 1;
+            rec.ext_lo = uint32_t(lo - std::min(lo, top.i0));
+            rec.ext_hi = uint32_t(std::max(hi, bottom.i1) - hi);
+        }
+        job.records.push_back(rec);
+        for (uint32_t part = 0; part < groups; part++) {
+            const uint32_t k_begin = part * chunks / groups, k_end = (part + 1) * chunks / groups;
+            MainStart st{0, 0};
+            if (k_begin < k_end) {
+                st.ymin = win_ymin[k_begin] - (k_begin == 0 ? int(rec.ext_lo) : 0);
+                st.slots = (win_slots[k_begin] & 0x7fffffffu) + (k_begin == 0 ? rec.ext_lo : 0u) + (k_begin == chunks - 1 ? rec.ext_hi : 0u);
+            }
+            job.starts.push_back(st);
+        }
+    }
+    raster_runs(j.items, 0, j.items.size(), job.args);
+}
+
 static void plan_main(const bt_preprocessor* p, const JobPlan& j, PlanOut& out) {
     FusedJobDev job = main_job(j);
 #ifdef BT_DEBUG_HOOKS
@@ -2337,6 +2512,7 @@
     }
     Launch lm = job_launch(j, kLaunchFusedMain, size_main_window(p, j, job.args));
     job.args.rotate_priority = 1;
+    build_main_records(p, j, lm.variant, job);
     lm.kernels = lm.variant == BT_VARIANT_MAIN_UNSTAGED ? 2u : 1u;
     lm.task_count = uint32_t(j.items.size());
     lm.aux0 = uint32_t(out.state.jobs.size());
@@ -2473,21 +2649,44 @@
 }
 
 static bt_status fused_upload(FusedState& state, const std::vector<std::vector<MainItem>>& items, const std::vector<std::vector<uint32_t>>& grids) {
+    struct Piece {
+        const void* host;
+        size_t bytes, at;
+    };
+    std::vector<Piece> pieces;
+    size_t bytes = 0;
+    auto add = [&](const void* host, size_t n) {
+        const size_t at = (bytes + 255) & ~size_t(255);
+        pieces.push_back({host, n, at});
+        bytes = at + n;
+        return at;
+    };
     std::vector<size_t> at(2 * items.size());
-    size_t bytes = 0;
-    for (size_t k = 0; k < at.size(); k++) {
-        at[k] = (bytes + 255) & ~size_t(255);
-        bytes = at[k] + (k % 2 ? grids[k / 2].size() * sizeof(uint32_t) : items[k / 2].size() * sizeof(MainItem));
+    for (size_t k = 0; k < items.size(); k++) {
+        at[2 * k] = add(items[k].data(), items[k].size() * sizeof(MainItem));
+        at[2 * k + 1] = add(grids[k].data(), grids[k].size() * sizeof(uint32_t));
+    }
+    std::vector<size_t> main_at(3 * state.jobs.size());
+    for (size_t k = 0; k < state.jobs.size(); k++) {
+        const FusedJobDev& job = state.jobs[k];
+        main_at[3 * k] = add(job.records.data(), job.records.size() * sizeof(MainRecord));
+        main_at[3 * k + 1] = add(job.starts.data(), job.starts.size() * sizeof(MainStart));
+        main_at[3 * k + 2] = add(job.tables.data(), job.tables.size());
     }
     BT_HIP(hipMalloc(&state.arrays, bytes ? bytes : 1));
     uint8_t* base = (uint8_t*)state.arrays;
-    for (size_t k = 0; k < items.size(); k++) {
-        if (!items[k].empty()) BT_HIP(hipMemcpy(base + at[2 * k], items[k].data(), items[k].size() * sizeof(MainItem), hipMemcpyHostToDevice));
-        if (!grids[k].empty()) BT_HIP(hipMemcpy(base + at[2 * k + 1], grids[k].data(), grids[k].size() * sizeof(uint32_t), hipMemcpyHostToDevice));
-    }
-    for (FusedJobDev& job : state.jobs) {
+    for (const Piece& piece : pieces)
+        if (piece.bytes) BT_HIP(hipMemcpy(base + piece.at, piece.host, piece.bytes, hipMemcpyHostToDevice));
+    for (size_t k = 0; k < state.jobs.size(); k++) {
+        FusedJobDev& job = state.jobs[k];
         job.args.items = (const MainItem*)(base + at[2 * job.queue_job]);
         job.args.grids = (const uint32_t*)(base + at[2 * job.queue_job + 1]);
+        job.args.records = (const MainRecord*)(base + main_at[3 * k]);
+        job.args.starts = (const MainStart*)(base + main_at[3 * k + 1]);
+        job.args.tables = base + main_at[3 * k + 2];
+        std::vector<MainRecord>().swap(job.records);
+        std::vector<MainStart>().swap(job.starts);
+        std::vector<uint8_t>().swap(job.tables);
     }
     return BT_OK;
 }
@@ -2653,6 +2852,11 @@
     A.rasters = p->rasters_dev;
     if ((l.kind == kLaunchFusedMain || l.kind == kLaunchFusedDirect) && item_begin < A.item_count) {
         A.items += item_begin;
+        if (l.kind == kLaunchFusedMain) {
+            A.records += item_begin;
+            A.starts += size_t(item_begin) * A.groups;
+            if (item_begin != 0) raster_runs(job.host_items, item_begin, item_count, A);
+        }
         A.item_count = std::min(item_count, A.item_count - item_begin);
     }
     const hipStream_t stream = p->ctx->stream;
```

Measured after the change: 4.731 million tiles/s, median of 6. Within noise of the previous version (+1.0%).
